# xiaopuren/KMC-with-a-diffusion-reaction-algorithm

Hardware: AMD Instinct MI355X
Metric: KMC particle-updates/sec (and steps/sec) at 1e6 particles, 1/2/4/8 MI355X (higher is better)
Workload: dtype f64

## Files before the change

kmc-with-a-diffusion-reaction-algorithm_amd/csrc/kmc_device.h:

```cpp
#pragma once
#include <hip/hip_runtime.h>
#include <stdint.h>

#include "kmc_math.h"
#include "kmc_philox.h"

namespace kmcd {

struct KParams {
  int NA, NB, N;
  int ncx, ncy;
  double gx0, gy0, cs;
  double box_x, box_y, box_z, pai;
  double ra, rb;
  double amp_a, amp_b, amp_cis, amp_bond;
  double rot_a, rot_b, rot_cis, rot_bond;
  double p_ass, p_mono, p_cis, p_diss, p_mdiss, p_cdiss;
  double bond_cut, cis_cut, thetapd_cut, thetaot_cut, cis_theta_cut;
  double T_aa, T_ab, T_bb, T_bond, T_cis;
  float ref_bb, ref_ab;
  int col_refine;
  float ref_rl;
  int rxn_refine;
  kmcr::Key key;
  int tcap;
  int tile;
  int dbg_stage;
  int tout_cap;
  int cx_serial;
  uint32_t cx_limit;
  int htag_max;
  int dbg_recs;
  int dbg_cand;
  int dd;
};

struct Ctl {
  uint32_t step;
  uint32_t obs_idx;
  uint32_t err;
  uint32_t err_step;
  uint32_t err_first;
  uint32_t n_overflow;
  uint32_t cx_cursor;
  uint32_t n_pend;
  uint32_t n_pqu, n_pqe;
  uint32_t n_cx;
  uint32_t n_heavy;
  uint32_t full_now;
  uint32_t n_dirty[2];
  uint32_t last[8];
  uint32_t n_rl;
  uint32_t n_cisc;
  uint32_t n_outl;
  uint32_t n_dense;
  int32_t off_bond, off_rl, off_cis, off_mono;
  int32_t maxc;
  uint32_t n_forced;
  uint32_t last_outl;
  uint32_t cand_kind[6];
  uint32_t rxn_kind[5];
  uint64_t vtag;
  uint64_t stamps[24];
  uint32_t dd_xcol, dd_xbond;
};

#define DD_JCAP 256
#define DD_XCAP 64
struct DDRep {
  int64_t xcol, xbond;
  int32_t bad, differed, links, n_jump, n_xb, reserved;
  int32_t jump_id[DD_JCAP];
  double jump_x[DD_JCAP];
  int32_t xb[DD_XCAP][2];
};

enum : uint32_t {
  ERR_EDGES = 1u,
  ERR_GEOMETRY = 2u,
  ERR_RESOLVE = 4u,
  ERR_ALIGN = 8u,
  ERR_MEMBERS = 16u,
  ERR_RECORDS = 32u,
};

enum : uint8_t { U_NONE = 0, U_FREE_A = 1, U_DIMER = 2, U_FREE_B = 3, U_COMPLEX = 4, U_DIMER_P = 5 };
enum : uint32_t { S_ACC = 1, S_PEND = 2, S_REJ = 3 };

#define ROWS_A 24
#define ROWS_B 12
#ifndef BEAD_BLOCK
#define BEAD_BLOCK 1
#endif
#ifndef BEAD_BS
#define BEAD_BS 64
#endif
#ifndef ROW_PERM
#define ROW_PERM 0
#endif
__host__ __device__ __forceinline__ int bead_row(int r, int rows) {
#if ROW_PERM
  constexpr unsigned char PA[24] = {0, 6, 7, 8, 1, 9, 10, 11, 2, 12, 13, 14, 3, 15, 16, 17, 4, 18, 19, 20, 5, 21, 22, 23};
  constexpr unsigned char PB[12] = {0, 6, 1, 7, 2, 8, 3, 9, 4, 10, 5, 11};
  return rows == 24 ? PA[r] : PB[r];
#else
  (void)rows;
  return r;
#endif
}
__host__ __device__ __forceinline__ size_t bead_elem(int i, int r, int n, int rows) {
#if BEAD_BLOCK
  (void)n;
  return ((size_t)(i / BEAD_BS) * rows + bead_row(r, rows)) * BEAD_BS + (i % BEAD_BS);
#else
  (void)rows;
  return (size_t)r * n + i;
#endif
}
__host__ __device__ __forceinline__ size_t bead_slots(int n) {
  return BEAD_BLOCK ? ((size_t)n + 63) / 64 * 64 : (size_t)n;
}
__host__ __device__ __forceinline__ size_t bead_off_a(int i, int j, int k, int c, int NA) {
  const int row = c < 2 ? (j - 1) * 4 + (k - 1) : 16 + ((j - 1) >> 1) * 4 + (k - 1);
  const int half = c < 2 ? c : ((j - 1) & 1);
  return bead_elem(i, row, NA, ROWS_A) * 2 + half;
}
__host__ __device__ __forceinline__ size_t bead_off_b(int i, int j, int k, int c, int NB) {
  const int row = c < 2 ? (j - 1) * 2 + (k - 1) : 8 + ((j - 1) >> 1) * 2 + (k - 1);
  const int half = c < 2 ? c : ((j - 1) & 1);
  return bead_elem(i, row, NB, ROWS_B) * 2 + half;
}
struct Beads {
  double* a;
  double* b;
  int NA, NB;
  __device__ __forceinline__ double& A(int i, int j, int k, int c) const { return a[bead_off_a(i, j, k, c, NA)]; }
  __device__ __forceinline__ double& B(int i, int j, int k, int c) const { return b[bead_off_b(i, j, k, c, NB)]; }
  __device__ __forceinline__ double2& A2(int i, int row) const {
    return reinterpret_cast<double2*>(a)[bead_elem(i, row, NA, ROWS_A)];
  }
  __device__ __forceinline__ double2& B2(int i, int row) const {
    return reinterpret_cast<double2*>(b)[bead_elem(i, row, NB, ROWS_B)];
  }
  __device__ __forceinline__ double2 Axy(int i, int j, int k) const { return A2(i, (j - 1) * 4 + (k - 1)); }
  __device__ __forceinline__ double2 Bxy(int i, int j, int k) const { return B2(i, (j - 1) * 2 + (k - 1)); }
  __device__ __forceinline__ double& P(int p, int j, int k, int c) const {
    return p < NA ? A(p, j, k, c) : B(p - NA, j, k, c);
  }
};

struct Rot {
  double t[3][3];
};
__device__ __forceinline__ Rot euler(double theta, double phi, double psai) {
  double cth = kmcm::cos(theta), sth = kmcm::sin(theta);
  double cph = kmcm::cos(phi), sph = kmcm::sin(phi);
  double cps = kmcm::cos(psai), sps = kmcm::sin(psai);
  Rot r;
  r.t[0][0] = cps * cph - cth * sph * sps;
  r.t[0][1] = -sps * cph - cth * sph * cps;
  r.t[0][2] = sth * sph;
  r.t[1][0] = cps * sph + cth * cph * sps;
  r.t[1][1] = -sps * sph + cth * cph * cps;
  r.t[1][2] = -sth * cph;
  r.t[2][0] = sps * sth;
  r.t[2][1] = cps * sth;
  r.t[2][2] = cth;
  return r;
}
__device__ __forceinline__ double rx(const Rot& r, double ox, double oy, double oz, double cx, double cy,
                                     double cz) {
  return r.t[0][0] * (ox - cx) + r.t[0][1] * (oy - cy) + r.t[0][2] * (oz - cz) + cx;
}
__device__ __forceinline__ double ry(const Rot& r, double ox, double oy, double oz, double cx, double cy,
                                     double cz) {
  return r.t[1][0] * (ox - cx) + r.t[1][1] * (oy - cy) + r.t[1][2] * (oz - cz) + cy;
}
__device__ __forceinline__ double rz(const Rot& r, double ox, double oy, double oz, double cx, double cy,
                                     double cz) {
  return r.t[2][0] * (ox - cx) + r.t[2][1] * (oy - cy) + r.t[2][2] * (oz - cz) + cz;
}

__device__ __forceinline__ double gettheta(double p0x, double p0y, double p0z, double p2x, double p2y,
                                           double p2z) {
  double lx0 = 0.0 - p0x, ly0 = 0.0 - p0y, lz0 = 0.0 - p0z;
  double lr0 = kmcm::sqrt_(lx0 * lx0 + ly0 * ly0 + lz0 * lz0);
  double lx1 = p2x - 0.0, ly1 = p2y - 0.0, lz1 = p2z - 0.0;
  double lr1 = kmcm::sqrt_(lx1 * lx1 + ly1 * ly1 + lz1 * lz1);
  double conv = 180 / 3.14159;
  double doth1 = -(lx1 * lx0 + ly0 * ly1 + lz0 * lz1);
  double doth2 = doth1 / (lr1 * lr0);
  if (doth2 > 1) doth2 = 1;
  if (doth2 < -1) doth2 = -1;
  return kmcm::acos(doth2) * conv;
}

__device__ __forceinline__ bool AreSame(double a, double b) { return kmcm::fabs_(a - b) < 1.0E-8; }

__device__ __forceinline__ double d2(double dx, double dy, double dz) { return dx * dx + dy * dy + dz * dz; }

__device__ __forceinline__ uint32_t ld_state(const uint32_t* p) {
  return __hip_atomic_load(p, __ATOMIC_RELAXED, __HIP_MEMORY_SCOPE_AGENT);
}
__device__ __forceinline__ void st_state(uint32_t* p, uint32_t v) {
  __hip_atomic_store(p, v, __ATOMIC_RELAXED, __HIP_MEMORY_SCOPE_AGENT);
}

}
```

kmc-with-a-diffusion-reaction-algorithm_amd/csrc/kmc_engine.hip:

```cpp
#include <hip/hip_runtime.h>

#include <algorithm>
#include <cmath>
#include <cstdio>
#include <cstdlib>
#include <cstring>
#include <string>
#include <vector>

#include "../../include/kmc.h"
#include "kmc_host.h"
#include "kmc_kernels.hip"
#include "kmc_analysis.hip"
#include "kmc_geometry.hip"
#include "kmc_structure.hip"
#include "kmc_dynamics.hip"

using namespace kmcd;

enum KId {
  KI_CLASSIFY, KI_BFS, KI_PROPOSE, KI_PROPOSE_FREE, KI_MOVE_MEMBERS, KI_CX_CHECK, KI_CX_HEAVY, KI_CX_KILL,
  KI_PAIR_SCAN, KI_COL_EXACT, KI_COL_ROUNDS, KI_COMMIT, KI_MATCH, KI_DISS_OBSERVE,
  KI_RESORT, KI_N
};
// ... 205 lines not shown
  rc |= dalloc(s, &d.dense, d.dense_cap);
  return rc;
}

double sqrt_threshold(double c) {
  double t = c * c;
  while (std::sqrt(t) >= c) t = std::nextafter(t, 0.0);
  while (std::sqrt(t) < c) t = std::nextafter(t, INFINITY);
  return t;
}


}

extern "C" {

const char* kmc_last_error(const kmc_sim* s) { return s ? s->err.c_str() : "null handle"; }

static int choose_tile(double rho) {
  int t = TILE_MAX;
  while (t > 4 && (t * t * rho > 205.0 || (t + 2) * (t + 2) * 2.0 * rho > 0.75 * TCAP)) --t;
  const char* te = getenv("KMC_TILE");
  if (te && *te) t = std::max(2, std::min(TILE_MAX, atoi(te)));
  return t;
}

int kmc_create(const kmc_params* p, int device, kmc_sim** out) {
  if (!p || !out) return KMC_ERR_ARG;
  *out = nullptr;
  if (p->n_a < 0 || p->n_b < 0 || p->n_a + p->n_b <= 0 || (int64_t)p->n_a + p->n_b > (1 << 24))
    return KMC_ERR_ARG;
  int ndev = 0;
  if (hipGetDeviceCount(&ndev) != hipSuccess || ndev == 0) return KMC_ERR_NODEVICE;
  kmc_sim* s = new kmc_sim();
  s->p = *p;
  if (device >= 0) {
    if (hipSetDevice(device) != hipSuccess) {
      delete s;
      return KMC_ERR_NODEVICE;
    }
    s->device = device;
  } else {
    (void)hipGetDevice(&s->device);
  }
  hipDeviceProp_t prop;
  if (hipGetDeviceProperties(&prop, s->device) != hipSuccess || std::strncmp(prop.gcnArchName, "gfx950", 6) != 0) {
    delete s;
    return KMC_ERR_NODEVICE;
  }
  if (hipStreamCreateWithFlags(&s->stream, hipStreamNonBlocking) != hipSuccess) {
    kmc_destroy(s);
    return KMC_ERR_HIP;
  }
  if (p->ra_radius > 20.0 || p->rb_radius > 30.0 || p->bond_dist_cutoff > 18.0 || p->cis_dist_cutoff > 15.0) {
    kmc_destroy(s);
    return KMC_ERR_ARG;
  }
  KParams& K = s->K;
  const int NA = p->n_a, NB = p->n_b, N = NA + NB;
  K.NA = NA;
  K.NB = NB;
  K.N = N;
  K.cs = 130.0;
  K.gx0 = -p->box_x / 2 - 1000.0;
  K.gy0 = -p->box_y / 2 - 1000.0;
  K.ncx = std::max(1, (int)((p->box_x + 2000.0) / K.cs) + 1);
  K.ncy = std::max(1, (int)((p->box_y + 2000.0) / K.cs) + 1);
  K.box_x = p->box_x;
  K.box_y = p->box_y;
  K.box_z = p->box_z;
  K.pai = p->pai;
  K.ra = p->ra_radius;
  K.rb = p->rb_radius;
  const double ts = p->time_step;
  K.amp_a = 2 * std::sqrt(p->ra_D * ts / 6);
  K.amp_b = 2 * std::sqrt(p->rb_D * ts / 6);
  K.amp_cis = 2 * std::sqrt(p->cis_D * ts / 6);
  K.amp_bond = 2 * std::sqrt(p->bond_D * ts / 6);
  K.rot_a = std::sqrt(p->ra_rot_D * ts);
  K.rot_b = std::sqrt(p->rb_rot_D * ts);
  K.rot_cis = std::sqrt(p->cis_rot_D * ts);
  K.rot_bond = std::sqrt(p->bond_rot_D * ts);
  K.p_ass = p->ass_rate * ts;
  K.p_mono = p->mono_cis_ass_rate * ts;
  K.p_cis = p->cis_ass_rate * ts;
  K.p_diss = p->diss_rate * ts;
  K.p_mdiss = p->mono_cis_diss_rate * ts;
  K.p_cdiss = p->cis_diss_rate * ts;
  K.bond_cut = p->bond_dist_cutoff;
  K.cis_cut = p->cis_dist_cutoff;
  K.thetapd_cut = p->bond_thetapd_cutoff;
  K.thetaot_cut = p->bond_thetaot_cutoff;
  K.cis_theta_cut = p->cis_thetaot_cutoff;
  K.T_aa = sqrt_threshold(p->ra_radius + p->ra_radius);
  K.T_ab = sqrt_threshold(p->ra_radius + p->rb_radius);
  K.T_bb = sqrt_threshold(p->rb_radius + p->rb_radius);
  K.T_bond = sqrt_threshold(p->bond_dist_cutoff);
  K.T_cis = sqrt_threshold(p->cis_dist_cutoff);
  K.ref_bb = (float)((2 * p->rb_radius + 2.5) * (2 * p->rb_radius + 2.5));
  K.ref_ab = (float)((p->ra_radius + p->rb_radius + 0.3 + 2.5) * (p->ra_radius + p->rb_radius + 0.3 + 2.5));
  K.ref_rl = (float)((p->bond_dist_cutoff + 3.0) * (p->bond_dist_cutoff + 3.0));
  {
    const char* cr = getenv("KMC_COL_REFINE");
    K.col_refine = !(cr && *cr == '0');
  }
  K.key = kmcr::make_key(p->seed, p->replica);

  s->ncell = 2 * K.ncx * K.ncy;
  Dev& d = s->d;
  d.cur.NA = d.nxt.NA = NA;
  d.cur.NB = d.nxt.NB = NB;
  d.nkeys = (uint32_t)N;
  int rc = KMC_OK;
  rc |= dalloc(s, &d.cur.a, 48 * bead_slots(NA));
  rc |= dalloc(s, &d.nxt.a, 48 * bead_slots(NA));
  rc |= dalloc(s, &d.cur.b, 24 * bead_slots(NB));
  rc |= dalloc(s, &d.nxt.b, 24 * bead_slots(NB));
  rc |= dalloc(s, &d.a_int, (size_t)5 * NA);
  rc |= dalloc(s, &d.b_int, (size_t)8 * NB);
  rc |= dalloc(s, &d.owner, N);
  rc |= dalloc(s, &d.id_of, N);
  rc |= dalloc(s, &d.slot_of, N);
  rc |= dalloc(s, &s->id_tmp, N);
  rc |= dalloc(s, &s->a_tmp, (size_t)5 * NA);
  rc |= dalloc(s, &s->b_tmp, (size_t)8 * NB);
  rc |= dalloc(s, &s->skeys, N);
  rc |= dalloc(s, &s->skeys2, N);
  rc |= dalloc(s, &s->svals, N);
  rc |= dalloc(s, &s->svals2, N);
  rc |= dalloc(s, &s->perm, N);
  rc |= dalloc(s, &s->newslot, N);
  rc |= dalloc(s, &d.ukind, N);
  rc |= dalloc(s, &d.ustate, N);
  rc |= dalloc(s, &d.moved, N);
  rc |= dalloc(s, &d.cx_off, NB);
  rc |= dalloc(s, &d.cx_size, NB);
  rc |= dalloc(s, &d.cx_nb, NB);
  rc |= dalloc(s, &d.cx_ext, NB);
  d.mcap = (uint32_t)(3 * (size_t)N);
  K.cx_limit = d.mcap / 2;
  {
    const char* cl = getenv("KMC_DEBUG_CX_LIMIT");
    if (cl && *cl) K.cx_limit = (uint32_t)std::max(0, std::min((int)K.cx_limit, atoi(cl)));
  }
  rc |= dalloc(s, &d.members, d.mcap);
  rc |= dalloc(s, &d.shuf, d.mcap);
  rc |= dalloc(s, &d.mrec, d.mcap);
  rc |= dalloc(s, &d.cxp, (size_t)NB * CXP);
  rc |= dalloc(s, &d.shuf_tag, NB);
  rc |= dalloc(s, &d.croot, N);
  rc |= dalloc(s, &d.cx_alive, NB);
  rc |= dalloc(s, &d.bfs_cand, NB);
  rc |= dalloc(s, &d.dlist, 2 * (size_t)N);
  rc |= dalloc(s, &d.pend, N);
  rc |= dalloc(s, &d.ccnt, N);
  rc |= dalloc(s, &d.overflow, NB);
  rc |= dalloc(s, &d.cx_list, (size_t)d.mcap / 2);
  rc |= dalloc(s, &d.cx_heavy, NB);
  rc |= dalloc(s, &s->hcnt, s->ncell + 1);
  {
    const size_t nblk = ((size_t)N + RS_TILE - 1) / RS_TILE;
    rc |= dalloc(s, &s->rs_cnt, 256 * nblk);
    rc |= dalloc(s, &s->rs_tot, 256);
    rc |= dalloc(s, &s->scan_part, ((size_t)s->ncell + 1 + SCAN_TILE - 1) / SCAN_TILE);
  }
  rc |= dalloc(s, &d.hstart, s->ncell + 1);
  rc |= dalloc(s, &d.home, N);
  rc |= dalloc(s, &d.rec, (size_t)2 * N);
  rc |= dalloc(s, &d.shard_cnt, (size_t)5 * NSHARD);
  {
    const char* cs = getenv("KMC_DEBUG_CAP_SHIFT");
    s->grow = cs && *cs ? -std::max(0, std::min(20, atoi(cs))) : 0;
  }
  rc |= alloc_lists(s);
  rc |= dalloc(s, &d.pq_units, N);
  rc |= dalloc(s, &d.obs_part, (size_t)8 * ((N + 255) / 256));
  rc |= dalloc(s, &d.bfs_queue, N);
  rc |= dalloc(s, &d.vtag, N);
  rc |= dalloc(s, &d.ctl, 1);
  if (rc != KMC_OK) {
    kmc_destroy(s);
    return KMC_ERR_HIP;
  }
  if (hipHostMalloc((void**)&s->ctl_host, sizeof(Ctl)) != hipSuccess) {
    kmc_destroy(s);
    return KMC_ERR_HIP;
  }
  const char* po = getenv("KMC_DEBUG_POISON");
  s->poison = po && *po == '1';
  const char* dc = getenv("KMC_DEBUG_COUNTS");
  s->debug_counts = dc && *dc == '1';
  const char* dsy = getenv("KMC_DEBUG_SYNC");
  s->debug_sync = dsy && *dsy == '1';
  const char* pc = getenv("KMC_DEBUG_PAIR_CHUNK");
  if (pc && *pc) s->an_chunk = std::max(1, std::min(AN_CHUNK, atoi(pc)));
  const char* tc = getenv("KMC_DEBUG_TCAP");
  K.tcap = TCAP;
  if (tc && *tc) K.tcap = std::max(0, std::min(TCAP, atoi(tc)));
  const char* oc = getenv("KMC_DEBUG_TOUT_CAP");
  K.tout_cap = TOUT_CAP;
  if (oc && *oc) K.tout_cap = std::max(0, std::min(TOUT_CAP, atoi(oc)));
  {
    K.tile = choose_tile((double)N * K.cs * K.cs / std::max(1.0, p->box_x * p->box_y));
    const char* fb = getenv("KMC_FULL_BFS");
    s->always_full = fb && *fb == '1';
    const char* ds = getenv("KMC_DEBUG_SCAN_STAGE");
    K.dbg_stage = ds && *ds ? atoi(ds) : 0;
    const char* cxs = getenv("KMC_CX_SERIAL");
    K.cx_serial = cxs && *cxs == '1';
    const char* gr = getenv("KMC_GRAPH");
    s->use_graphs = gr && *gr == '1';
    const char* cs = getenv("KMC_CX_STREAM");
    s->cx_stream = (cs && *cs) ? std::max(0, std::min(3, atoi(cs))) : ((int64_t)N >= CX_STREAM_N ? 3 : 0);
    const char* cpw = getenv("KMC_CX_PARAMS_WG");
    s->cx_params_wg = cpw && *cpw ? std::max(0, atoi(cpw)) : 0;
    const char* ht = getenv("KMC_DEBUG_HTAG");
    K.htag_max = HTAG_MAX;
    if (ht && *ht) K.htag_max = std::max(0, std::min(HTAG_MAX, atoi(ht)));
    const char* dca = getenv("KMC_DEBUG_CAND");
    K.dbg_cand = dca && *dca == '1';
    const char* dr = getenv("KMC_DEBUG_RECS");
    K.dbg_recs = dr && *dr == '1';
    if (K.dbg_recs && dalloc(s, &d.rec_step, 2 * (size_t)N) != KMC_OK) {
      kmc_destroy(s);
      return KMC_ERR_HIP;
    }
    const char* sp = getenv("KMC_SNAP_SPAN");
    if (sp && *sp) s->snap_span = std::max<int64_t>(0, atoll(sp));
  }
  {
    const uint64_t kmax = (uint64_t)K.ncx * K.ncy;
    s->key_bits = 1;
    while ((1ull << s->key_bits) < kmax) ++s->key_bits;
    if (s->key_bits + 33 > 64) {
      kmc_destroy(s);
      return KMC_ERR_ARG;
    }
    const char* re = getenv("KMC_RESORT");
    if (re && *re) s->resort_every = atoll(re);
    const char* gs = getenv("KMC_GROUP_SORT");
    if (gs && *gs) s->group_sort = std::max(0, std::min(2, atoi(gs)));
    s->ntiles = ((K.ncx + K.tile - 1) / K.tile) * ((K.ncy + K.tile - 1) / K.tile);
    if (dalloc(s, &s->d.tout, (size_t)s->ntiles * TOUT_CAP) != KMC_OK ||
        dalloc(s, &s->d.tout_n, (size_t)s->ntiles) != KMC_OK) {
      kmc_destroy(s);
      return KMC_ERR_HIP;
    }
  }
  *out = s;
  return KMC_OK;
}

int kmc_destroy(kmc_sim* s) {
  if (!s) return KMC_OK;
  if (s->stream) (void)hipStreamSynchronize(s->stream);
  for (void* v : s->allocs) (void)hipFree(v);
  if (s->obs_buf) (void)hipFree(s->obs_buf);
  if (s->ctl_host) (void)hipHostFree(s->ctl_host);
  for (auto& e : s->tev)
    if (e) (void)hipEventDestroy(e);
  for (auto& g : s->graphs)
    if (g.exec) (void)hipGraphExecDestroy(g.exec);
  if (s->side) (void)hipStreamSynchronize(s->side);
  for (auto& e : s->an_ev)
    if (e) (void)hipEventDestroy(e);
  if (s->ev_fork) (void)hipEventDestroy(s->ev_fork);
  if (s->ev_join) (void)hipEventDestroy(s->ev_join);
  if (s->side) (void)hipStreamDestroy(s->side);
  if (s->stream) (void)hipStreamDestroy(s->stream);
  delete s;
  return KMC_OK;
}

int64_t kmc_current_step(const kmc_sim* s) { return s ? s->step_done : -1; }

static void reorder(kmc_sim* s, const int32_t* perm, const int32_t* map, bool swap_in) {
  const KParams& K = s->K;
  Dev& d = s->d;
  hipStream_t st = s->stream;
  const int NA = K.NA, NB = K.NB, T = 256, mode = swap_in ? 0 : 1;
  auto g = [&](size_t n) { return (unsigned)((n + T - 1) / T); };
  if (NA > 0) {
    k_gather_beads<<<g((size_t)(swap_in ? ROWS_A : 48) * NA), T, 0, st>>>(d.cur.a, d.nxt.a, perm, 0, NA, 0, mode);
    k_gather_i32<<<g((size_t)5 * NA), T, 0, st>>>(d.a_int, s->a_tmp, perm, 0, NA, 5, (1u << 2) | (1u << 4), map);
  }
  if (NB > 0) {
    k_gather_beads<<<g((size_t)(swap_in ? ROWS_B : 24) * NB), T, 0, st>>>(d.cur.b, d.nxt.b, perm, NA, NB, 1, mode);
    k_gather_i32<<<g((size_t)8 * NB), T, 0, st>>>(d.b_int, s->b_tmp, perm, NA, NB, 8, 0xf0u, map);
  }
  if (!swap_in) return;
  std::swap(d.cur.a, d.nxt.a);
  std::swap(d.cur.b, d.nxt.b);
  std::swap(d.a_int, s->a_tmp);
  std::swap(d.b_int, s->b_tmp);
}

__global__ void k_iota(int32_t* a, int32_t* b, int n) {
  int i = blockIdx.x * blockDim.x + threadIdx.x;
  if (i < n) a[i] = b[i] = i;
}

static void dev_scan(kmc_sim* s, const int32_t* in, int32_t* out, int n, hipStream_t st) {
  const int nb = (n + SCAN_TILE - 1) / SCAN_TILE;
  k_scan_part<<<nb, 256, 0, st>>>(in, n, s->scan_part);
  k_scan_top<<<1, 256, 0, st>>>(s->scan_part, nb);
  k_scan_down<<<nb, 256, 0, st>>>(in, out, n, s->scan_part);
}

static int32_t* radix_sort(kmc_sim* s, int nbits, hipStream_t st, uint64_t** keys_out) {
  const int N = s->K.N, nblk = (N + RS_TILE - 1) / RS_TILE;
  uint64_t *ka = s->skeys, *kb = s->skeys2;
  int32_t *va = s->svals, *vb = s->svals2;
  if (nblk == 0) nbits = 0;
  for (int shift = 0; shift < nbits; shift += 8) {
    k_rs_hist<<<nblk, 256, 0, st>>>(ka, N, shift, s->rs_cnt, nblk);
    k_rs_rows<<<256, 256, 0, st>>>(s->rs_cnt, nblk, s->rs_tot);
    k_rs_scatter<<<nblk, 256, 0, st>>>(ka, va, kb, vb, N, shift, s->rs_cnt, s->rs_tot, nblk);
    std::swap(ka, kb);
    std::swap(va, vb);
  }
  *keys_out = ka;
  return va;
}

static int check_sort(kmc_sim* s, const uint64_t* dk, const int32_t* dv) {
  const int N = s->K.N, NA = s->K.NA;
  std::vector<uint64_t> k((size_t)N);
  std::vector<int32_t> v((size_t)N);
  HIPCHK(s, hipStreamSynchronize(s->stream));
  HIPCHK(s, hipMemcpy(k.data(), dk, sizeof(uint64_t) * N, hipMemcpyDeviceToHost));
  HIPCHK(s, hipMemcpy(v.data(), dv, sizeof(int32_t) * N, hipMemcpyDeviceToHost));
  std::vector<uint8_t> seen((size_t)N, 0);
  for (int i = 0; i < N; ++i) {
    const int kind = i >= NA, base = kind ? NA : 0, nk = kind ? N - NA : NA;
    if (v[i] < 0 || v[i] >= nk || seen[(size_t)base + v[i]]++)
      return fail(s, KMC_ERR_HIP, "KMC_DEBUG_SYNC: re-sort values not a permutation at " + std::to_string(i));
    if (i > 0 && (k[i] < k[i - 1] || (k[i] == k[i - 1] && v[i] <= v[i - 1])))
      return fail(s, KMC_ERR_HIP, "KMC_DEBUG_SYNC: re-sort keys out of order at " + std::to_string(i));
  }
  return KMC_OK;
}

static int home_build(kmc_sim* s) {
  const KParams& K = s->K;
  Dev& d = s->d;
  hipStream_t st = s->stream;
  const int N = K.N, T = 256;
  HIPCHK(s, hipMemsetAsync(s->hcnt, 0, sizeof(int32_t) * (size_t)(s->ncell + 1), st));
  k_home_count<<<(N + T - 1) / T, T, 0, st>>>(K, d, s->hcnt);
  dev_scan(s, s->hcnt, d.hstart, s->ncell + 1, st);
  if (s->debug_sync) {
    const size_t n = (size_t)s->ncell + 1;
    std::vector<int32_t> c(n), h(n);
    HIPCHK(s, hipStreamSynchronize(st));
    HIPCHK(s, hipMemcpy(c.data(), s->hcnt, sizeof(int32_t) * n, hipMemcpyDeviceToHost));
    HIPCHK(s, hipMemcpy(h.data(), d.hstart, sizeof(int32_t) * n, hipMemcpyDeviceToHost));
    int64_t run = 0;
    for (size_t i = 0; i < n; ++i) {
      if (h[i] != run) return fail(s, KMC_ERR_HIP, "KMC_DEBUG_SYNC: home scan wrong at " + std::to_string(i));
      run += c[i];
    }
  }
  k_home_place<<<(N + T - 1) / T, T, 0, st>>>(K, d);
  return hipGetLastError() == hipSuccess ? KMC_OK : fail(s, KMC_ERR_HIP, "home_build launch");
}

// ... 188 lines not shown

int kmc_load_cpt(kmc_sim* s, const char* path) {
  if (!s || !path) return KMC_ERR_ARG;
  const int NA = s->p.n_a, NB = s->p.n_b;
  std::vector<double> ra((size_t)48 * NA + 1), rb((size_t)24 * NB + 1);
  std::vector<int32_t> ai((size_t)5 * NA + 1), bi((size_t)8 * NB + 1);
  kmc_state_view v{ra.data(), rb.data(), ai.data(), bi.data(), {0, 0, 0, 0, 0}, 0, 0};
  int rc = kmch_host::load_cpt(&s->p, path, &v, &s->err);
  if (rc != KMC_OK) return rc;
  return kmc_set_state(s, &v);
}

int kmc_write_cpt(kmc_sim* s, const char* path) {
  if (!s || !path) return KMC_ERR_ARG;
  const int NA = s->p.n_a, NB = s->p.n_b;
  std::vector<double> ra((size_t)48 * NA + 1), rb((size_t)24 * NB + 1);
  std::vector<int32_t> ai((size_t)5 * NA + 1), bi((size_t)8 * NB + 1);
  kmc_state_view v{ra.data(), rb.data(), ai.data(), bi.data(), {0, 0, 0, 0, 0}, 0, 0};
  int rc = kmc_get_state(s, &v);
  if (rc != KMC_OK) return rc;
  return kmch_host::write_cpt(&s->p, &v, path, &s->err);
}

int kmc_save_state(kmc_sim* s, const char* path) {
  if (!s || !path) return KMC_ERR_ARG;
  const int NA = s->p.n_a, NB = s->p.n_b;
  std::vector<double> ra((size_t)48 * NA + 1), rb((size_t)24 * NB + 1);
  std::vector<int32_t> ai((size_t)5 * NA + 1), bi((size_t)8 * NB + 1);
  kmc_state_view v{ra.data(), rb.data(), ai.data(), bi.data(), {0, 0, 0, 0, 0}, 0, 0};
  int rc = kmc_get_state(s, &v);
  if (rc != KMC_OK) return rc;
  return kmch_host::save_state(&s->p, &v, path, &s->err);
}

int kmc_load_state(kmc_sim* s, const char* path) {
  if (!s || !path) return KMC_ERR_ARG;
  const int NA = s->p.n_a, NB = s->p.n_b;
  std::vector<double> ra((size_t)48 * NA + 1), rb((size_t)24 * NB + 1);
  std::vector<int32_t> ai((size_t)5 * NA + 1), bi((size_t)8 * NB + 1);
  kmc_state_view v{ra.data(), rb.data(), ai.data(), bi.data(), {0, 0, 0, 0, 0}, 0, 0};
  int rc = kmch_host::load_state(&s->p, path, &v, &s->err);
  if (rc != KMC_OK) return rc;
  return kmc_set_state(s, &v);
}

static void harvest(kmc_sim* s, int slot) {
  for (int k = 0; k < KI_N; ++k) {
    size_t i = (size_t)slot * KI_N + k;
    if (!s->tused[i]) continue;
    float ms = 0;
    (void)hipEventSynchronize(s->tev[2 * i + 1]);
    if (hipEventElapsedTime(&ms, s->tev[2 * i], s->tev[2 * i + 1]) == hipSuccess) {
      s->kms[k] += ms;
      s->kcount[k] += 1;
    }
    s->tused[i] = 0;
  }
}

struct Bracket {
  kmc_sim* s;
  int k;
  hipStream_t st;
  Bracket(kmc_sim* s_, int k_, hipStream_t st_) : s(s_), k(k_), st(st_) {
    if (s->tnow && (s->tmask >> k & 1)) (void)hipEventRecord(s->tev[2 * ((size_t)s->tslot * KI_N + k)], st);
  }
  ~Bracket() {
    if (s->tnow && (s->tmask >> k & 1)) {
      size_t i = (size_t)s->tslot * KI_N + k;
      (void)hipEventRecord(s->tev[2 * i + 1], st);
      s->tused[i] = 1;
    }
  }
};
#define TIMED(k, ...) TIMED_ON(k, s->stream, __VA_ARGS__)
#define TIMED_ON(k, STREAM, ...)                                                                        \
  do {                                                                                                  \
    {                                                                                                   \
      Bracket b_(s, k, STREAM);                                                                         \
      __VA_ARGS__;                                                                                      \
    }                                                                                                   \
    if (s->debug_sync) {                                                                                \
      const hipError_t e_ = hipStreamSynchronize(STREAM);                                               \
      if (e_ != hipSuccess)                                                                             \
        return fail(s, KMC_ERR_HIP, std::string("KMC_DEBUG_SYNC: ") + KNAMES[k] + " failed in step " +     \
                                        std::to_string(s->launch_base) + ": " + hipGetErrorString(e_)); \
    }                                                                                                   \
  } while (0)

static int debug_check_lists(kmc_sim* s) {
  Dev& d = s->d;
  const int N = s->K.N;
  HIPCHK(s, hipStreamSynchronize(s->stream));
  std::vector<uint32_t> cnt(5 * NSHARD);
  HIPCHK(s, hipMemcpy(cnt.data(), d.shard_cnt, sizeof(uint32_t) * cnt.size(), hipMemcpyDeviceToHost));
  const SList* L[5] = {&d.cand, &d.conf, &d.plist, &d.rej, &d.pairs};
  const char* names[5] = {"cand", "conf", "plist", "rej", "pairs"};
  char m[300];
  for (int l = 0; l < 5; ++l) {
    std::vector<int2> v((size_t)L[l]->cap * NSHARD);
    HIPCHK(s, hipMemcpy(v.data(), L[l]->data, sizeof(int2) * v.size(), hipMemcpyDeviceToHost));
    for (int k = 0; k < NSHARD; ++k) {
      const uint32_t c = std::min(cnt[l * NSHARD + k], L[l]->cap);
      for (uint32_t t = 0; t < c; ++t) {
        const int2 e = v[(size_t)k * L[l]->cap + t];
        const int x = e.x, y = l == 1 ? (e.y & 0x7fffffff) : e.y;
        bool ok = true;
        if (l == 0 || l == 4) ok = x >= 0 && x < 2 * N && y >= 0 && y < 2 * N;
        if (l == 1) ok = x >= 0 && x < N && y >= 0 && y < N;
        if (l == 2 || l == 3) ok = x >= 0 && x < N;
        if (!ok) {
          snprintf(m, sizeof m, "KMC_DEBUG_SYNC: list %s shard %d entry %u = (%d, %d) out of range (N %d) in step %lld",
                   names[l], k, t, e.x, e.y, N, (long long)s->launch_base);
          return fail(s, KMC_ERR_HIP, m);
        }
      }
    }
  }
  return KMC_OK;
}

#ifndef COARSE_N
#define COARSE_N (4 << 20)
#endif
static int side_stream(kmc_sim* s) {
  if (s->side) return KMC_OK;
  int lo = 0, hi = 0;
  const char* pr = getenv("KMC_CX_STREAM_PRIO");
  const bool prio = !(pr && *pr == '0') && hipDeviceGetStreamPriorityRange(&lo, &hi) == hipSuccess;
  if ((prio ? hipStreamCreateWithPriority(&s->side, hipStreamNonBlocking, hi)
            : hipStreamCreateWithFlags(&s->side, hipStreamNonBlocking)) != hipSuccess ||
      hipEventCreateWithFlags(&s->ev_fork, hipEventDisableTiming) != hipSuccess ||
      hipEventCreateWithFlags(&s->ev_join, hipEventDisableTiming) != hipSuccess)
    return fail(s, KMC_ERR_HIP, "the complexes' stream");
  return KMC_OK;
}

static int launch_step(kmc_sim* s, bool re_sort) {
  const KParams& K = s->K;
  Dev& d = s->d;
  hipStream_t st = s->stream;
  const int T = 256;
  const int gN = (K.N + T - 1) / T, gB = (K.NB + T - 1) / T;
  if (s->tnow) harvest(s, s->tslot);
  if (re_sort) {
    int rc;
    TIMED(KI_RESORT, rc = resort(s));
    if (rc != KMC_OK) return rc;
  }
  if (s->poison) {
    (void)hipMemsetAsync(d.nxt.a, 0xff, sizeof(double) * 48 * bead_slots(K.NA), st);
    (void)hipMemsetAsync(d.nxt.b, 0xff, sizeof(double) * 24 * bead_slots(K.NB), st);
  }
  if (K.NB > 0 && (s->need_full || re_sort || s->always_full))
    TIMED(KI_CX_KILL, (k_cx_kill<<<std::min(gN, 1024), T, 0, st>>>(K, d)));
  s->need_full = false;
  const int per = K.N >= COARSE_N ? 4 : 1, gP = (K.N + T * per - 1) / (T * per);
  if (per == 4) TIMED(KI_CLASSIFY, (k_classify<4><<<gP, T, 0, st>>>(K, d)));
  else TIMED(KI_CLASSIFY, (k_classify<1><<<gP, T, 0, st>>>(K, d)));
  {
    Bracket b_(s, KI_PROPOSE, st);
    const int gL = std::min(2048, (K.NB + T - 1) / T);
    const bool side = s->cx_stream != 0 && K.NB > 0 && !s->use_graphs;
    if (K.NB > 0 && (!side || s->cx_stream == 3)) {
      TIMED(KI_BFS, (k_bfs<<<gB, T, 0, st>>>(K, d)));
    }
    const int gC = K.NB > 0 ? std::min(gL, 512) : 0;
    const int gP3 = s->cx_params_wg > 0 ? std::min(s->cx_params_wg, 1 << 16) : gL;
    if (side && s->cx_stream == 3) {
      const int rc = side_stream(s);
      if (rc != KMC_OK) return rc;
      hipStream_t sd = s->side;
      k_propose_free<<<gP3, T, 0, st>>>(K, d, gP3);
      TIMED(KI_MOVE_MEMBERS, (k_move_members<<<gN, T, 0, st>>>(K, d)));
      HIPCHK(s, hipEventRecord(s->ev_fork, st));
      HIPCHK(s, hipStreamWaitEvent(sd, s->ev_fork, 0));
      TIMED_ON(KI_CX_CHECK, sd, (k_cx_check<<<gL, T, 0, sd>>>(K, d)));
      TIMED_ON(KI_CX_HEAVY, sd, (k_complex_heavy<<<1024, T, 0, sd>>>(K, d)));
      HIPCHK(s, hipEventRecord(s->ev_join, sd));
      TIMED(KI_PROPOSE_FREE, (k_propose_free<<<gN, T, 0, st>>>(K, d, 0)));
      HIPCHK(s, hipStreamWaitEvent(st, s->ev_join, 0));
    } else if (side) {
      const int rc = side_stream(s);
      if (rc != KMC_OK) return rc;
      hipStream_t sd = s->side;
      HIPCHK(s, hipEventRecord(s->ev_fork, st));
      HIPCHK(s, hipStreamWaitEvent(sd, s->ev_fork, 0));
      TIMED_ON(KI_BFS, sd, (k_bfs<<<gB, T, 0, sd>>>(K, d)));
      k_propose_free<<<gC, T, 0, sd>>>(K, d, gC);
      if (s->cx_stream == 1) {
        TIMED_ON(KI_MOVE_MEMBERS, sd, (k_move_members<<<gN, T, 0, sd>>>(K, d)));
        TIMED_ON(KI_CX_CHECK, sd, (k_cx_check<<<gL, T, 0, sd>>>(K, d)));
        TIMED_ON(KI_CX_HEAVY, sd, (k_complex_heavy<<<1024, T, 0, sd>>>(K, d)));
      }
      HIPCHK(s, hipEventRecord(s->ev_join, sd));
      TIMED(KI_PROPOSE_FREE, (k_propose_free<<<gN, T, 0, st>>>(K, d, 0)));
      HIPCHK(s, hipStreamWaitEvent(st, s->ev_join, 0));
      if (s->cx_stream == 2) {
        TIMED(KI_MOVE_MEMBERS, (k_move_members<<<gN, T, 0, st>>>(K, d)));
        TIMED(KI_CX_CHECK, (k_cx_check<<<gL, T, 0, st>>>(K, d)));
        TIMED(KI_CX_HEAVY, (k_complex_heavy<<<1024, T, 0, st>>>(K, d)));
      }
    } else {
      TIMED(KI_PROPOSE_FREE, (k_propose_free<<<gC + gN, T, 0, st>>>(K, d, gC)));
      if (K.NB > 0) {
        TIMED(KI_MOVE_MEMBERS, (k_move_members<<<gN, T, 0, st>>>(K, d)));
        TIMED(KI_CX_CHECK, (k_cx_check<<<gL, T, 0, st>>>(K, d)));
        TIMED(KI_CX_HEAVY, (k_complex_heavy<<<1024, T, 0, st>>>(K, d)));
      }
    }
  }
  if (K.dbg_recs) k_rec_check<<<std::min(2048, (2 * K.N + T - 1) / T), T, 0, st>>>(K, d);
  const int gX = std::min(2048, (K.N + T - 1) / T);
  const int ntiles = s->ntiles;
  TIMED(KI_PAIR_SCAN, (k_pair_scan<<<ntiles, PAIR_THREADS, 0, st>>>(K, d)));
  TIMED(KI_COL_EXACT, {
#if DENSE_KERNEL
    k_col_dense<<<64, T, 0, st>>>(K, d);
    if (s->debug_sync && hipStreamSynchronize(st) != hipSuccess)
      return fail(s, KMC_ERR_HIP, "KMC_DEBUG_SYNC: k_col_dense failed in step " + std::to_string(s->launch_base));
#endif
    k_col_exact<<<std::max(gX, 64), T, 0, st>>>(K, d);
  });
  if (s->debug_sync) {
    const int rc = debug_check_lists(s);
    if (rc != KMC_OK) return rc;
  }
  TIMED(KI_COL_ROUNDS, {
    k_col_resolve<<<gX, T, 0, st>>>(K, d);
    if (s->debug_sync && hipStreamSynchronize(st) != hipSuccess)
      return fail(s, KMC_ERR_HIP, "KMC_DEBUG_SYNC: k_col_resolve failed in step " + std::to_string(s->launch_base));
    k_col_tail<<<1, 1024, 0, st>>>(K, d, 1);
  });
#ifndef COMMIT_RXN
#define COMMIT_RXN 1
#endif
#if COMMIT_RXN
  TIMED(KI_COMMIT, (k_commit_rxn<<<gX + (K.NA > 0 ? 1024 : 0), T, 0, st>>>(K, d, gX)));
#else
  TIMED(KI_COMMIT, {
    k_commit_rxn<<<gX, T, 0, st>>>(K, d, gX);
    if (K.NA > 0) k_commit_rxn<<<1024, T, 0, st>>>(K, d, 0);
  });
#endif
  if (K.NA > 0) TIMED(KI_MATCH, (k_match<<<1, 1024, 0, st>>>(K, d)));
  TIMED(KI_DISS_OBSERVE, {
    if (per == 4) k_diss_observe<4><<<gP, T, 0, st>>>(K, d);
    else k_diss_observe<1><<<gP, T, 0, st>>>(K, d);
    k_finalize<<<1, 1024, 0, st>>>(K, d, s->p.time_step, gP);
  });
  if (s->tnow) s->tslot = (s->tslot + 1) % TRING;
  std::swap(d.cur, d.nxt);
  return KMC_OK;
}

static int launch_step_graph(kmc_sim* s) {
  unsigned char key[sizeof(KParams) + sizeof(Dev)];
  std::memcpy(key, &s->K, sizeof(KParams));
  std::memcpy(key + sizeof(KParams), &s->d, sizeof(Dev));
  for (auto& g : s->graphs)
    if (g.valid && std::memcmp(g.key, key, sizeof key) == 0) {
      HIPCHK(s, hipGraphLaunch(g.exec, s->stream));
      std::swap(s->d.cur, s->d.nxt);
      ++s->graph_launches;
      return KMC_OK;
    }
  auto& g = s->graphs[s->graph_next];
  s->graph_next = (s->graph_next + 1) % kmc_sim::NGRAPH;
  if (g.exec) (void)hipGraphExecDestroy(g.exec);
  g.exec = nullptr;
  g.valid = false;
  HIPCHK(s, hipStreamBeginCapture(s->stream, hipStreamCaptureModeThreadLocal));
  const int rc = launch_step(s, false);
  hipGraph_t graph = nullptr;
  const hipError_t ec = hipStreamEndCapture(s->stream, &graph);
  if (rc != KMC_OK) {
    if (graph) (void)hipGraphDestroy(graph);
    return rc;
  }
  HIPCHK(s, ec);
  const hipError_t ei = hipGraphInstantiate(&g.exec, graph, nullptr, nullptr, 0);
  (void)hipGraphDestroy(graph);
  HIPCHK(s, ei);
  std::memcpy(g.key, key, sizeof key);
  g.valid = true;
  ++s->graph_captures;
  HIPCHK(s, hipGraphLaunch(g.exec, s->stream));
  ++s->graph_launches;
  return KMC_OK;
}

static int dd_after_step(kmc_sim* s);

static int run_chunk(kmc_sim* s, int64_t n, int64_t base, kmc_obs* out = nullptr) {
  HIPCHK(s, hipMemsetAsync(&s->d.ctl->obs_idx, 0, sizeof(uint32_t), s->stream));
  for (int64_t k = 0; k < n; ++k) {
    const bool rs = s->resort_every > 0 && ++s->since_resort >= s->resort_every;
    if (rs) s->since_resort = 0;
    if (((base + k + 1) & 0x3fffffff) == 0)
      HIPCHK(s, hipMemsetAsync(s->d.ustate, 0, sizeof(uint32_t) * (size_t)s->K.N, s->stream));
    s->tnow = s->tmask && (s->tcount++ % s->tperiod) == 0;
    const bool plain = !rs && !s->tnow && !s->poison && !s->need_full && !s->always_full &&
                       s->K.dbg_stage == 0 && !s->debug_sync;
    s->launch_base = base + k + 1;
    int rc = (s->use_graphs && plain) ? launch_step_graph(s) : launch_step(s, rs);
    if (rc != KMC_OK) return rc;
  }
  HIPCHK(s, hipGetLastError());
  if (s->dd_step_pending) {
    const int rc = dd_after_step(s);
    if (rc != KMC_OK) return rc;
  }
  HIPCHK(s, hipMemcpyAsync(s->ctl_host, s->d.ctl, sizeof(Ctl), hipMemcpyDeviceToHost, s->stream));
  if (out) HIPCHK(s, hipMemcpyAsync(out, s->obs_buf, sizeof(kmc_obs_dev) * n, hipMemcpyDeviceToHost, s->stream));
  HIPCHK(s, hipStreamSynchronize(s->stream));
  if (s->tmask)
    for (int slot = 0; slot < TRING; ++slot) harvest(s, slot);
  return KMC_OK;
}

int kmc_step(kmc_sim* s, int64_t nsteps, kmc_obs* out) {
  if (!s) return KMC_ERR_ARG;
  if (!s->have_state) return fail(s, KMC_ERR_ARG, "no state: call kmc_init_random / kmc_load_cpt / kmc_set_state");
  if (nsteps <= 0) return KMC_OK;
  static_assert(sizeof(kmc_obs_dev) == sizeof(kmc_obs), "obs layout");
  const int64_t chunk = 4096;
  if (!s->obs_buf) {
    HIPCHK(s, hipMalloc((void**)&s->obs_buf, sizeof(kmc_obs_dev) * chunk));
    s->obs_cap = chunk;
    s->d.obs = s->obs_buf;
  }
  int64_t done = 0;
  while (done < nsteps) {
    const int64_t n = std::min(chunk, nsteps - done);
    int rc = KMC_OK;
    if (!s->K.dd && (!s->snap_valid || s->step_done + n - s->snap_step > s->snap_span)) {
      rc = snapshot(s, false);
      if (rc != KMC_OK) return rc;
      s->snap_valid = true;
      s->snap_step = s->step_done;
      s->snap_since = s->since_resort;
      ++s->n_snapshots;
    }
    bool copied = false;
    for (;;) {
      rc = run_chunk(s, n, s->step_done, out ? out + done : nullptr);
      if (rc != KMC_OK) return rc;
      const uint32_t err = s->ctl_host->err;
      if (!err) {
        copied = out != nullptr;
        break;
      }
      const uint32_t cause = s->ctl_host->err_first;
      const int64_t bad = (int64_t)s->ctl_host->err_step;
      if (s->K.dd) {
        const bool grow = (cause & ~ERR_EDGES) == 0;
        if (grow && s->grow < 6) {
          s->grow += 1;
          if (alloc_lists(s) != KMC_OK) return fail(s, KMC_ERR_HIP, "growing the output lists failed");
        }
        s->have_state = false;
        s->clusters_valid = false;
        char m[200];
        snprintf(m, sizeof m, "dd: device error bits 0x%x at step %lld; the window's state is lost (list growth 2^%d)",
                 err, (long long)bad, s->grow);
        return fail(s, grow ? KMC_ERR_CAPACITY : (cause & ERR_GEOMETRY) ? KMC_ERR_GEOMETRY : KMC_ERR_CAPACITY, m);
      }
      rc = snapshot(s, true);
      if (rc != KMC_OK) return rc;
      s->since_resort = s->snap_since;
      s->need_full = true;
      ++s->n_replays;
      const bool grow = (cause & ~ERR_EDGES) == 0 && s->grow < 6;
      if (grow) {
        s->grow += 1;
        if (alloc_lists(s) != KMC_OK) return fail(s, KMC_ERR_HIP, "growing the output lists failed");
      }
      for (int64_t at = s->snap_step; at < s->step_done;) {
        const int64_t m = std::min(chunk, s->step_done - at);
        rc = run_chunk(s, m, at);
        if (rc != KMC_OK) return rc;
        if (s->ctl_host->err) {
          rc = snapshot(s, true);
          if (rc != KMC_OK) {
            s->have_state = false;
            return rc;
          }
          const int64_t at_fail = at;
          s->step_done = s->snap_step;
          s->since_resort = s->snap_since;
          s->need_full = true;
          s->clusters_valid = false;
          char m2[200];
          snprintf(m2, sizeof m2,
                   "replay from the snapshot raised an error the original steps did not (in steps %lld..%lld); "
                   "state restored to step %lld",
                   (long long)at_fail + 1, (long long)(at_fail + m), (long long)s->step_done);
          return fail(s, KMC_ERR_HIP, m2);
        }
        at += m;
      }
      if (grow) continue;
      const int64_t good = std::max<int64_t>(0, std::min<int64_t>(n, bad - (s->step_done + 1)));
      if (good > 0) {
        rc = run_chunk(s, good, s->step_done);
        if (rc != KMC_OK) return rc;
        if (out)
          HIPCHK(s, hipMemcpy(out + done, s->obs_buf, sizeof(kmc_obs_dev) * good, hipMemcpyDeviceToHost));
        s->step_done += good;
      }
      s->clusters_valid = good > 0;
      char m[200];
      snprintf(m, sizeof m, "device error bits 0x%x at step %lld; state kept at step %lld", err, (long long)bad,
               (long long)s->step_done);
      const int code = (cause & ERR_GEOMETRY) ? KMC_ERR_GEOMETRY : KMC_ERR_CAPACITY;
      return fail(s, code, m);
    }
    if (out && !copied)
      HIPCHK(s, hipMemcpy(out + done, s->obs_buf, sizeof(kmc_obs_dev) * n, hipMemcpyDeviceToHost));
    s->step_done += n;
    s->clusters_valid = true;
    if (s->debug_counts) {
      const uint32_t* l = s->ctl_host->last;
      fprintf(stderr, "kmc step %lld: candidates %u conflicts %u pending-units %u rejected %u rxn-pairs %u rl-edges %u cis-edges %u bfs-overflow %u outliers %u (list growth 2^%d, replays %lld, snapshots %lld, forced rebuilds %u)\n",
              (long long)s->step_done, l[0], l[1], l[2], l[3], l[4], l[5], l[6], l[7], s->ctl_host->last_outl, s->grow,
              (long long)s->n_replays, (long long)s->n_snapshots, s->ctl_host->n_forced);
      if (s->K.dbg_cand) {
        const uint32_t* c = s->ctl_host->cand_kind;
        const uint32_t* r = s->ctl_host->rxn_kind;
        fprintf(stderr, "kmc cand AA %u/%u AB %u/%u BB %u/%u (tested/colliding) rxn %u final %u gate %u accept %u "
                "refined-out %u\n",
                c[0], c[1], c[2], c[3], c[4], c[5], r[0], r[1], r[2], r[3], r[4]);
      }
#if WALK_STATS
      {
        unsigned long long w = 0, wo = 0;
        if (hipMemcpyFromSymbol(&w, HIP_SYMBOL(kmc_walk_pairs), sizeof w) == hipSuccess &&
            hipMemcpyFromSymbol(&wo, HIP_SYMBOL(kmc_walk_pairs_old), sizeof wo) == hipSuccess)
          fprintf(stderr, "kmc walk pairs %llu old-position items %llu (summed since the library loaded)\n", w, wo);
      }
#endif
      const uint64_t* t = s->ctl_host->stamps;
      if (t[16])
        fprintf(stderr, "kmc stamps heavy stage %llu align %llu writeback %llu records %llu (cycles summed over "
                "waves) complexes %llu max-cycles %llu members %llu\n",
                (unsigned long long)t[16], (unsigned long long)t[17], (unsigned long long)t[18],
                (unsigned long long)t[19], (unsigned long long)t[20], (unsigned long long)t[21],
                (unsigned long long)t[22]);
      if (t[0] | t[8])
        fprintf(stderr, "kmc stamps col %llu %llu %llu %llu %llu %llu %llu %llu rxn %llu %llu %llu %llu %llu %llu %llu %llu\n",
                (unsigned long long)t[0], (unsigned long long)t[1], (unsigned long long)t[2], (unsigned long long)t[3],
                (unsigned long long)t[4], (unsigned long long)t[5], (unsigned long long)t[6], (unsigned long long)t[7],
                (unsigned long long)t[8], (unsigned long long)t[9], (unsigned long long)t[10], (unsigned long long)t[11],
                (unsigned long long)t[12], (unsigned long long)t[13], (unsigned long long)t[14], (unsigned long long)t[15]);
    }
    done += n;
  }
  return KMC_OK;
}

__global__ void k_math(int op, const double* x, const double* y, double* out, int n) {
  int i = blockIdx.x * blockDim.x + threadIdx.x;
  if (i >= n) return;
  double a = x[i], b = y[i], r = 0;
  switch (op) {
    case 0: r = kmcm::sin(a); break;
    case 1: r = kmcm::cos(a); break;
    case 2: r = kmcm::atan2(a, b); break;
    case 3: r = kmcm::acos(a); break;
    case 4: r = kmcm::sqrt_(a); break;
    case 5: r = a / b; break;
    default: r = kmcm::round_(a); break;
  }
  out[i] = r;
}

int kmc_device_math(int op, const double* x, const double* y, double* out, int64_t n) {
  if (n <= 0) return KMC_OK;
  double *dx = nullptr, *dy = nullptr, *dout = nullptr;
  size_t b = sizeof(double) * (size_t)n;
  if (hipMalloc(&dx, b) != hipSuccess || hipMalloc(&dy, b) != hipSuccess || hipMalloc(&dout, b) != hipSuccess)
    return KMC_ERR_HIP;
  int rc = KMC_OK;
  if (hipMemcpy(dx, x, b, hipMemcpyHostToDevice) != hipSuccess || hipMemcpy(dy, y, b, hipMemcpyHostToDevice) != hipSuccess)
    rc = KMC_ERR_HIP;
  if (rc == KMC_OK) {
    k_math<<<(int)((n + 255) / 256), 256>>>(op, dx, dy, dout, (int)n);
    if (hipDeviceSynchronize() != hipSuccess || hipMemcpy(out, dout, b, hipMemcpyDeviceToHost) != hipSuccess)
      rc = KMC_ERR_HIP;
  }
  (void)hipFree(dx);
  (void)hipFree(dy);
  (void)hipFree(dout);
  return rc;
}

int kmc_get_clusters(kmc_sim* s, int32_t* row_len, int32_t* members) {
  if (!s || !row_len || !members) return KMC_ERR_ARG;
  if (!s->have_state || !s->clusters_valid)
    return fail(s, KMC_ERR_ARG, "no step simulated since the state was set (or the last chunk was undone)");
  const int NA = s->p.n_a, NB = s->p.n_b, N = NA + NB;
  std::vector<uint8_t> kind(N);
  std::vector<int32_t> off(NB), size(NB), mem(N), id_of(N), slot_of(N);
  HIPCHK(s, hipStreamSynchronize(s->stream));
  HIPCHK(s, hipMemcpy(kind.data(), s->d.ukind, N, hipMemcpyDeviceToHost));
  HIPCHK(s, hipMemcpy(off.data(), s->d.cx_off, sizeof(int32_t) * NB, hipMemcpyDeviceToHost));
  HIPCHK(s, hipMemcpy(size.data(), s->d.cx_size, sizeof(int32_t) * NB, hipMemcpyDeviceToHost));
  std::vector<int32_t> shuf(s->d.mcap);
  std::vector<uint32_t> stag(NB);
  mem.resize(s->d.mcap);
  HIPCHK(s, hipMemcpy(mem.data(), s->d.members, sizeof(int32_t) * s->d.mcap, hipMemcpyDeviceToHost));
  HIPCHK(s, hipMemcpy(shuf.data(), s->d.shuf, sizeof(int32_t) * s->d.mcap, hipMemcpyDeviceToHost));
  HIPCHK(s, hipMemcpy(stag.data(), s->d.shuf_tag, sizeof(uint32_t) * NB, hipMemcpyDeviceToHost));
  HIPCHK(s, hipMemcpy(id_of.data(), s->d.id_of, sizeof(int32_t) * N, hipMemcpyDeviceToHost));
  HIPCHK(s, hipMemcpy(slot_of.data(), s->d.slot_of, sizeof(int32_t) * N, hipMemcpyDeviceToHost));
  int64_t o = 0;
  for (int b = 0; b < NB; ++b) {
    int p = slot_of[NA + b];
    if (kind[p] == U_FREE_B) {
      row_len[b] = 1;
      members[o++] = NA + b + 1;
    } else if (kind[p] == U_COMPLEX) {
      int lb = p - NA;
      row_len[b] = size[lb];
      const int32_t* row = (stag[lb] == (uint32_t)s->step_done ? shuf.data() : mem.data()) + off[lb];
      for (int t = 0; t < size[lb]; ++t) members[o++] = id_of[row[t]] + 1;
    } else {
      row_len[b] = 0;
    }
  }
  return KMC_OK;
}

int kmc_set_timing(kmc_sim* s, uint64_t kernel_mask) {
  if (!s) return KMC_ERR_ARG;
  if (kernel_mask && s->tev.empty()) {
    s->tev.assign((size_t)TRING * KI_N * 2, nullptr);
    s->tused.assign((size_t)TRING * KI_N, 0);
    for (auto& e : s->tev) HIPCHK(s, hipEventCreate(&e));
  }
  s->tmask = kernel_mask;
  s->tcount = 0;
  for (int k = 0; k < KI_N; ++k) {
    s->kms[k] = 0;
    s->kcount[k] = 0;
  }
  return KMC_OK;
}

int kmc_set_timing_period(kmc_sim* s, int32_t every) {
  if (!s || every < 1) return KMC_ERR_ARG;
  s->tperiod = every;
  return KMC_OK;
}

int kmc_kernel_times(const kmc_sim* s, double* total_ms, int64_t* launches, int32_t n) {
  if (!s) return KMC_ERR_ARG;
  for (int k = 0; k < n && k < KI_N; ++k) {
    if (total_ms) total_ms[k] = s->kms[k];
    if (launches) launches[k] = s->kcount[k];
  }
  return KI_N;
}

const char* kmc_kernel_name(int32_t id) { return id >= 0 && id < KI_N ? KNAMES[id] : ""; }

}

__global__ void k_dd_export(KParams P, Dev d, int n, const int32_t* ids, double* beads, int32_t* ints) {
  const int NA = P.NA, NB = P.NB;
  const size_t t = (size_t)blockIdx.x * blockDim.x + threadIdx.x;
  if (t < (size_t)n * 48) {
    const int i = (int)(t / 48), e = (int)(t % 48), slot = d.slot_of[ids[i]], bead = e / 3, c = e % 3;
    double v = 0.0;
    if (slot < NA) v = d.cur.A(slot, bead / 4 + 1, bead % 4 + 1, c);
    else if (e < 24) v = d.cur.B(slot - NA, bead / 2 + 1, bead % 2 + 1, c);
    beads[t] = v;
  }
  if (t < (size_t)n * 8) {
    const int i = (int)(t / 8), f = (int)(t % 8), slot = d.slot_of[ids[i]];
    int v = 0;
    bool link = false;
    if (slot < NA) {
      if (f < 5) v = d.a_int[(size_t)f * NA + slot];
      link = f == 2 || f == 4;
    } else {
      v = d.b_int[(size_t)f * NB + (slot - NA)];
      link = f >= 4;
    }
    if (link && v > 0) v = d.id_of[v - 1] + 1;
    ints[t] = v;
  }
}

__global__ void k_dd_import(KParams P, Dev d, int n, const int32_t* ids, const double* beads, const int32_t* ints,
                            uint8_t* flags) {
  const int NA = P.NA, NB = P.NB;
  const size_t t = (size_t)blockIdx.x * blockDim.x + threadIdx.x;
  if (t < (size_t)n * 48) {
    const int i = (int)(t / 48), e = (int)(t % 48), slot = d.slot_of[ids[i]], bead = e / 3, c = e % 3;
    double* dst = nullptr;
    if (slot < NA) dst = &d.cur.A(slot, bead / 4 + 1, bead % 4 + 1, c);
    else if (e < 24) dst = &d.cur.B(slot - NA, bead / 2 + 1, bead % 2 + 1, c);
    if (dst) {
      const double v = beads[t];
      if (__double_as_longlong(*dst) != __double_as_longlong(v)) {
        atomicOr((uint32_t*)&flags[i & ~3], 1u << (8 * (i & 3)));
        *dst = v;
      }
    }
  }
  if (t < (size_t)n * 8) {
    const int i = (int)(t / 8), f = (int)(t % 8), slot = d.slot_of[ids[i]];
    int32_t* dst = nullptr;
    bool link = false;
    if (slot < NA) {
      if (f < 5) dst = &d.a_int[(size_t)f * NA + slot];
      link = f == 2 || f == 4;
    } else {
      dst = &d.b_int[(size_t)f * NB + (slot - NA)];
      link = f >= 4;
    }
    if (dst) {
      int v = ints[t];
      if (link && v > 0) v = d.slot_of[v - 1] + 1;
      if (*dst != v) {
        atomicOr((uint32_t*)&flags[i & ~3], 2u << (8 * (i & 3)));
        *dst = v;
      }
    }
  }
}

__global__ void k_dd_drift(KParams P, Dev d, uint32_t* out) {
  const int p = blockIdx.x * blockDim.x + threadIdx.x;
  float m = 0.0f;
  if (p < P.N) {
    const int r = d.id_of[p];
    if (d.dd_own[r]) {
      double dx = d.cur.P(p, 1, 1, 0) - d.dd_x0[r];
      dx = dx - P.box_x * kmcm::round_(dx / P.box_x);
      m = (float)kmcm::fabs_(dx);
    }
  }
  for (int o = 32; o > 0; o >>= 1) m = fmaxf(m, __shfl_down(m, o, 64));
  if (__lane_id() == 0) atomicMax(out, __float_as_uint(m));
}

__global__ void k_dd_jumpers(KParams P, Dev d, double S, int cap, int32_t* ids, double* xs, uint32_t* cnt) {
  const int p = blockIdx.x * blockDim.x + threadIdx.x;
  if (p >= P.N) return;
  const int r = d.id_of[p];
  if (!d.dd_own[r]) return;
  const double x = d.cur.P(p, 1, 1, 0);
  double dx = x - d.dd_x0[r];
  dx = dx - P.box_x * kmcm::round_(dx / P.box_x);
  if (!(kmcm::fabs_(dx) > S)) return;
  const uint32_t k = atomicAdd(cnt, 1u);
// ... 989 lines not shown
```

kmc-with-a-diffusion-reaction-algorithm_amd/csrc/kmc_kernels.hip:

```cpp
#include "kmc_device.h"

namespace kmcd {

#ifndef NSHARD
#define NSHARD 64
#endif
struct SList {
  int2* data;
  uint32_t* cnt;
  uint32_t cap;
};

struct Dev {
  Beads cur, nxt;
  int32_t* a_int;
  int32_t* b_int;
  int32_t* owner;
  int32_t* id_of;
  int32_t* slot_of;
  uint8_t* ukind;
  uint32_t* ustate;
  uint32_t* moved;
  int32_t* cx_off;
  int32_t* cx_size;
  int32_t* cx_nb;
  uint32_t* cx_ext;
  int32_t* members;
  int32_t* shuf;
  int4* mrec;
  double* cxp;
  uint32_t* shuf_tag;
  uint32_t mcap;
  int32_t* croot;
  uint32_t* cx_alive;
  uint32_t* bfs_cand;
  int32_t* dlist;
  uint32_t* pend;
  unsigned long long* ccnt;
  int32_t* overflow;
  int4* cx_list;
  int4* cx_heavy;
  uint2* home;
  int32_t* hstart;
  struct Rec* rec;
  int4* outl;
  uint32_t outl_cap;
  int2* tout;
  uint32_t* tout_n;
  uint32_t* rec_step;
  int4* dense;
  uint32_t dense_cap;
  SList cand;
  SList conf;
  SList plist;
  SList rej;
  SList pairs;
  int32_t* pq_units;
  int2* pq_ent;
  uint32_t* shard_cnt;
  int32_t* obs_part;
  uint64_t* rl_keys;
  uint64_t* cis_keys;
  uint64_t* ent;
  int32_t* gi32;
  uint32_t cap_edges;
  int32_t* bfs_queue;
  uint32_t* vtag;
  Ctl* ctl;
  struct kmc_obs_dev* obs;
  const int32_t* gid;
  const uint8_t* dd_own;
  const double* dd_x0;
  DDRep* dd_rep;
  uint32_t nkeys;
};

struct alignas(16) Rec {
  float4 pos;
  int2 id;
  float2 site;
};
#define RID_PID 0x00ffffff
#define RID_LIG (1 << 24)
#define RID_CODE_SHIFT 25
#define RID_OUT 15
#define RID_ST3 (1 << 29)
#define RID_ST2 (1 << 30)
__device__ __forceinline__ int rec_code(int2 id) { return (id.x >> RID_CODE_SHIFT) & 15; }

struct kmc_obs_dev {
  int64_t step;
  double t;
  int32_t rl, mono, cis, bond;
  double cluster_size;
  int32_t maxc, tot_prot, tot_clu, reserved;
};

#define A_ST2(d, i) (d).a_int[0 * (size_t)NA + (i)]
#define A_ST3(d, i) (d).a_int[1 * (size_t)NA + (i)]
#define A_NEI2(d, i) (d).a_int[2 * (size_t)NA + (i)]
#define A_NEI4(d, i) (d).a_int[3 * (size_t)NA + (i)]
#define A_NEI3(d, i) (d).a_int[4 * (size_t)NA + (i)]
#define B_ST(d, b, j) (d).b_int[(size_t)((j)-1) * NB + (b)]
#define B_NEI(d, b, j) (d).b_int[(size_t)(4 + (j)-1) * NB + (b)]

__device__ __forceinline__ bool bad_key(const Dev& d, int key) {
  if ((uint32_t)key < d.nkeys) return false;
  atomicOr(&d.ctl->err, ERR_RESOLVE);
  return true;
}
__device__ __forceinline__ uint32_t state_of(const Dev& d, int key, uint32_t step) {
  if (bad_key(d, key)) return S_REJ;
  uint32_t v = ld_state(&d.ustate[key]);
  return (v >> 2) == (step & 0x3fffffffu) ? (v & 3u) : S_ACC;
}
__device__ __forceinline__ void set_state(const Dev& d, int key, uint32_t step, uint32_t s) {
  if (bad_key(d, key)) return;
  st_state(&d.ustate[key], ((step & 0x3fffffffu) << 2) | s);
}

__device__ __forceinline__ uint32_t rkey(const KParams& P, const Dev& d, int r) {
  return P.dd ? (uint32_t)d.gid[r] : (uint32_t)r;
}
__device__ __forceinline__ bool dd_owned(const KParams& P, const Dev& d, int r) { return !P.dd || d.dd_own[r]; }
__device__ __forceinline__ void dd_xbond(const Dev& d, int a, int b) {
  if (d.dd_own[a] == d.dd_own[b]) return;
  atomicAdd(&d.ctl->dd_xbond, 1u);
  const uint32_t k = atomicAdd((uint32_t*)&d.dd_rep->n_xb, 1u);
  if (k < DD_XCAP) {
    d.dd_rep->xb[k][0] = a;
    d.dd_rep->xb[k][1] = b;
  }
}

__device__ __forceinline__ int cell_x(const KParams& P, double x) {
  int c = (int)__builtin_floor((x - P.gx0) / P.cs);
  return c < 0 ? 0 : (c >= P.ncx ? P.ncx - 1 : c);
}
__device__ __forceinline__ int cell_y(const KParams& P, double y) {
  int c = (int)__builtin_floor((y - P.gy0) / P.cs);
  return c < 0 ? 0 : (c >= P.ncy ? P.ncy - 1 : c);
}

#define CROOT_BIG (1 << 30)
#define CXL 16

__device__ __forceinline__ uint32_t wave_slot(uint32_t* ctr) {
  const uint64_t mask = __ballot(1);
  const int lane = __lane_id();
  const int leader = __ffsll((unsigned long long)mask) - 1;
  const uint32_t rank = __popcll(mask & ((1ull << lane) - 1ull));
  uint32_t base = 0;
  if (lane == leader) base = atomicAdd(ctr, (uint32_t)__popcll(mask));
  base = __shfl(base, leader, 64);
  return base + rank;
}

__device__ __forceinline__ uint32_t wave_alloc(uint32_t* ctr, uint32_t qn) {
  const uint64_t mask = __ballot(1);
  const int lane = __lane_id(), leader = __ffsll((unsigned long long)mask) - 1;
  uint32_t pre = 0, tot = 0;
  for (uint64_t m = mask; m; m &= m - 1) {
    const int l = __ffsll((unsigned long long)m) - 1;
    const uint32_t v = (uint32_t)__shfl((int)qn, l, 64);
    pre += l < lane ? v : 0u;
    tot += v;
  }
  uint32_t base = 0;
  if (lane == leader) base = atomicAdd(ctr, tot);
  return (uint32_t)__shfl((int)base, leader, 64) + pre;
}

template <int CLASSIFY_PER>
__global__ void k_classify(KParams P, Dev d) {
  const int NA = P.NA, NB = P.NB;
  const int p0 = blockIdx.x * blockDim.x * CLASSIFY_PER + threadIdx.x;
  int n2[CLASSIFY_PER], n3[CLASSIFY_PER], s2[CLASSIFY_PER], r[CLASSIFY_PER];
#pragma unroll
  for (int k = 0; k < CLASSIFY_PER; ++k) {
    const int p = p0 + k * (int)blockDim.x;
    n2[k] = n3[k] = s2[k] = 0;
    r[k] = -1;
    if (p >= P.N) continue;
    if (p < NA) {
      n2[k] = A_NEI2(d, p);
      n3[k] = A_NEI3(d, p);
      s2[k] = A_ST2(d, p) | A_ST3(d, p);
    } else {
      const int b = p - NA;
      n2[k] = B_NEI(d, b, 2);
      n3[k] = B_NEI(d, b, 3);
      s2[k] = B_NEI(d, b, 4);
    }
    r[k] = d.croot[p];
    if (r[k] >= 0) r[k] &= ~CROOT_BIG;
  }
#pragma unroll
  for (int k = 0; k < CLASSIFY_PER; ++k) {
    const int p = p0 + k * (int)blockDim.x;
    if (p >= P.N) continue;
    uint8_t kind = U_NONE;
    int own = -1;
    if (p < NA) {
      const int i = p;
      if (s2[k] == 0) {
        kind = U_FREE_A;
        own = p;
      } else if (n2[k] == 0 && n3[k] != 0 && A_NEI3(d, n3[k] - 1) == i + 1 && A_NEI2(d, n3[k] - 1) == 0) {
        int q = n3[k] - 1;
        const bool lead = d.id_of[i] < d.id_of[q];
        own = lead ? i : q;
        kind = lead ? U_DIMER : U_DIMER_P;
      }
    } else if (n2[k] == 0 && n3[k] == 0 && s2[k] == 0) {
      kind = U_FREE_B;
      own = p;
    }
    if (r[k] >= 0) {
      own = r[k];
      if (r[k] == p) kind = U_COMPLEX;
    }
    d.ukind[p] = kind;
    d.owner[p] = own < 0 ? -1 : d.id_of[own];
  }
}

__device__ __forceinline__ void cx_reset_all(const KParams& P, const Dev& d, uint32_t tid, uint32_t nt) {
  for (uint32_t p = tid; p < (uint32_t)P.N; p += nt) d.croot[p] = -1;
  for (uint32_t b = tid; b < (uint32_t)P.NB; b += nt) d.cx_alive[b] = 0;
  if (tid == 0) {
    d.ctl->cx_cursor = 0;
    d.ctl->n_cx = 0;
    d.ctl->full_now = 1;
  }
}
__global__ void k_cx_kill(KParams P, Dev d) {
  cx_reset_all(P, d, blockIdx.x * blockDim.x + threadIdx.x, gridDim.x * blockDim.x);
}
__device__ __forceinline__ void cx_dissolve_dirty(const KParams& P, const Dev& d, uint32_t step) {
  const int NA = P.NA;
  const uint32_t li = step & 1, n = min(d.ctl->n_dirty[li], (uint32_t)P.N), next = step + 1;
  for (uint32_t t = threadIdx.x; t < n; t += blockDim.x) {
    const int p = d.dlist[(size_t)li * P.N + t];
    if (p >= NA) d.bfs_cand[p - NA] = next;
    const int r = d.croot[p] & ~CROOT_BIG;
    if (r < 0 || atomicExch(&d.cx_alive[r - NA], 0u) != 1u) continue;
    const int b = r - NA, off = d.cx_off[b], sz = d.cx_size[b];
    for (int i = 0; i < sz; ++i) {
      const int m = d.members[off + i];
      d.croot[m] = -1;
      if (m >= NA) d.bfs_cand[m - NA] = next;
    }
  }
}

__device__ __forceinline__ void mark_bond_change(const KParams& P, const Dev& d, int p, uint32_t step) {
  if (P.NB == 0) return;
  const uint32_t li = step & 1;
  const uint32_t t = atomicAdd(&d.ctl->n_dirty[li], 1u);
  if (t < (uint32_t)P.N) d.dlist[(size_t)li * P.N + t] = p;
}

#define BFS_QCAP 32
#ifndef BFS_BATCH
#define BFS_BATCH 4
#endif

__device__ __forceinline__ void nbrs3(const KParams& P, const Dev& d, int x, int* y) {
  const int NA = P.NA, NB = P.NB;
  if (x < NA) {
    const int a = A_NEI2(d, x), b = A_NEI3(d, x);
    y[0] = a > 0 ? a - 1 : (b > 0 ? b - 1 : -1);
    y[1] = a > 0 && b > 0 ? b - 1 : -1;
    y[2] = -1;
  } else {
    const int lb = x - NA;
    const int v2 = B_NEI(d, lb, 2), v3 = B_NEI(d, lb, 3), v4 = B_NEI(d, lb, 4);
    y[0] = v2 > 0 ? v2 - 1 : -1;
    y[1] = v3 > 0 ? v3 - 1 : -1;
    y[2] = v4 > 0 ? v4 - 1 : -1;
  }
}

#define CXD_MOVED (1 << 30)
#define CXD_LB 0x3fffffff

template <int STRIDE = 1>
__device__ __forceinline__ void register_complex(const KParams& P, const Dev& d, int p, const int* q, int qn) {
  const int NA = P.NA, NB = P.NB;
  uint32_t off = wave_alloc(&d.ctl->cx_cursor, (uint32_t)qn);
  if (off + qn > d.mcap) {
    atomicOr(&d.ctl->err, ERR_MEMBERS);
    qn = 0;
    off = 0;
  }
  int nb = 0;
  const int rootid = d.id_of[p];
#pragma unroll 4
  for (int t = 0; t < qn; ++t) {
    int m = q[t * STRIDE];
    d.members[off + t] = m;
    d.owner[m] = rootid;
    d.croot[m] = p | (qn > CXL ? CROOT_BIG : 0);
    nb += m >= NA;
  }
  d.cx_alive[p - NA] = 1;
  if (qn <= CXL) {
    auto enc = [&](int v) -> int {
      if (v <= 0) return 0;
      for (int t = 0; t < qn; ++t)
        if (q[t * STRIDE] == v - 1) return (v - 1 < NA ? t : NA + t) + 1;
      atomicOr(&d.ctl->err, ERR_RESOLVE);
      return 0;
    };
    for (int t0 = 0; t0 < qn; t0 += 4) {
      int4 r[4];
#pragma unroll
      for (int i = 0; i < 4; ++i) {
        const int t = t0 + i, m = t < qn ? q[t * STRIDE] : p;
        r[i].x = m;
        if (m < NA) {
          r[i].y = A_NEI2(d, m);
          r[i].z = A_NEI3(d, m);
          r[i].w = A_NEI4(d, m);
        } else {
          r[i].y = B_NEI(d, m - NA, 2);
          r[i].z = B_NEI(d, m - NA, 3);
          r[i].w = B_NEI(d, m - NA, 4);
        }
      }
#pragma unroll
      for (int i = 0; i < 4; ++i) {
        if (t0 + i >= qn) break;
        r[i].y = enc(r[i].y);
        r[i].z = enc(r[i].z);
        if (r[i].x >= NA) r[i].w = enc(r[i].w);
        d.mrec[off + t0 + i] = r[i];
      }
    }
  }
  int b = p - NA;
  d.cx_off[b] = (int)off;
  d.cx_size[b] = qn;
  d.cx_nb[b] = nb;
  d.ukind[p] = U_COMPLEX;
  const int4 desc = make_int4(b, (int)off, qn | nb << 16, rootid);
  const uint32_t slot = wave_slot(&d.ctl->n_cx);
  if (slot < d.mcap / 2) d.cx_list[slot] = desc;
  else atomicOr(&d.ctl->err, ERR_MEMBERS);
}

__global__ void __launch_bounds__(256) k_bfs(KParams P, Dev d) {
  __shared__ int qs[BFS_QCAP * 256];
  const int NA = P.NA, NB = P.NB;
  int b = blockIdx.x * blockDim.x + threadIdx.x;
  if (b >= NB) return;
  if (!d.ctl->full_now && d.bfs_cand[b] != d.ctl->step) return;
  if (B_NEI(d, b, 2) == 0 && B_NEI(d, b, 3) == 0 && B_NEI(d, b, 4) == 0) return;
  int* q = qs + threadIdx.x;
  int p = NA + b;
  const int pid = d.id_of[p];
  auto lower = [&](int qn) {
    bool lw = false;
    for (int t0 = 1; t0 < qn; t0 += 8) {
      int id[8];
#pragma unroll
      for (int i = 0; i < 8; ++i) {
        const int t = t0 + i, v = t < qn ? q[t * 256] : 0;
        id[i] = v >= NA ? d.id_of[v] : pid;
      }
#pragma unroll
      for (int i = 0; i < 8; ++i) lw |= id[i] < pid;
    }
    return lw;
  };
  int qn = 1, head = 0;
  q[0] = p;
  uint64_t bloom = 1ull << (((uint32_t)p * 0x9E3779B1u) >> 26);
  while (head < qn) {
    const int nb = min(BFS_BATCH, qn - head);
    int y[BFS_BATCH][3];
#pragma unroll
    for (int i = 0; i < BFS_BATCH; ++i)
      if (i < nb) nbrs3(P, d, q[(head + i) * 256], y[i]);
#pragma unroll
    for (int i = 0; i < BFS_BATCH; ++i) {
      if (i >= nb) break;
#pragma unroll
      for (int e = 0; e < 3; ++e) {
        int v = y[i][e];
        if (v < 0) continue;
        const uint64_t bit = 1ull << (((uint32_t)v * 0x9E3779B1u) >> 26);
        if (bloom & bit) {
          bool seen = false;
          for (int t = 0; t < qn; ++t) seen |= q[t * 256] == v;
          if (seen) continue;
        }
        bloom |= bit;
        if (qn == BFS_QCAP) {
          if (lower(qn) || (v >= NA && d.id_of[v] < pid)) return;
          uint32_t s = atomicAdd(&d.ctl->n_overflow, 1u);
          d.overflow[s] = b;
          return;
        }
        q[(qn++) * 256] = v;
      }
    }
    head += nb;
  }
  if (lower(qn)) return;
  register_complex<256>(P, d, p, q, qn);
}

__device__ __forceinline__ int bfs_overflow_one(const KParams& P, const Dev& d, uint32_t o) {
  const int NA = P.NA;
  int p = NA + d.overflow[o];
  const int pid = d.id_of[p];
  uint32_t tag = (uint32_t)(++d.ctl->vtag);
  int* q = d.bfs_queue;
  int qn = 0, head = 0;
  q[qn++] = p;
  d.vtag[p] = tag;
  while (head < qn) {
    int x = q[head++];
    int y[3];
    nbrs3(P, d, x, y);
#pragma unroll
    for (int e = 0; e < 3; ++e) {
      int v = y[e];
      if (v < 0) continue;
      if (v >= NA && d.id_of[v] < pid) return -1;
      if (d.vtag[v] == tag) continue;
      d.vtag[v] = tag;
      q[qn++] = v;
    }
  }
  register_complex(P, d, p, q, qn);
  return p - NA;
}

typedef double kmc_dbl2v __attribute__((ext_vector_type(2)));
__device__ __forceinline__ double2 ld_r(const double2& r) {
  const kmc_dbl2v v = __builtin_nontemporal_load(reinterpret_cast<const kmc_dbl2v*>(&r));
  return make_double2(v.x, v.y);
}
__device__ __forceinline__ void st_n(double2& r, double2 v) {
  kmc_dbl2v w;
  w.x = v.x;
  w.y = v.y;
  __builtin_nontemporal_store(w, reinterpret_cast<kmc_dbl2v*>(&r));
}

__device__ __forceinline__ void ref_point(const Dev& d, const Beads& B, int p, int NA, double& x, double& y,
                                          double& zlo, double& zhi) {
  if (p < NA) {
    const double2 xy = B.Axy(p, 1, 1), z12 = B.A2(p, 16), z34 = B.A2(p, 20);
    x = xy.x;
    y = xy.y;
    double z1 = z12.x, z2 = z12.y, z3 = z34.x, z4 = z34.y;
    zlo = fmin(fmin(z1, z2), fmin(z3, z4));
    zhi = fmax(fmax(z1, z2), fmax(z3, z4));
  } else {
    const double2 xy = B.Bxy(p - NA, 1, 1);
    x = xy.x;
    y = xy.y;
    zlo = B.B(p - NA, 1, 1, 2);
    zhi = zlo;
  }
}

__device__ __forceinline__ bool extent_ok(const Beads& B, int p, int NA) {
  if (p < NA) {
    double x0 = B.A(p, 1, 1, 0), y0 = B.A(p, 1, 1, 1);
    for (int j = 2; j <= 4; ++j) {
      double dx = B.A(p, j, 1, 0) - x0, dy = B.A(p, j, 1, 1) - y0;
      if (!(dx * dx + dy * dy <= 0.09)) return false;
    }
    return true;
  }
  int b = p - NA;
  double x0 = B.B(b, 1, 1, 0), y0 = B.B(b, 1, 1, 1);
  for (int j = 2; j <= 4; ++j) {
    double dx = B.B(b, j, 1, 0) - x0, dy = B.B(b, j, 1, 1) - y0;
    if (!(dx * dx + dy * dy <= 35.0 * 35.0)) return false;
  }
  return true;
}

__device__ __forceinline__ int cell_index(const KParams& P, int cx, int cy, int kind) {
  return (cy * 2 + kind) * P.ncx + cx;
}

#ifndef TOUT_CAP
#define TOUT_CAP 64
#endif
__device__ __forceinline__ void tile_bucket_push(const KParams& P, const Dev& d, int ri, int cx, int cy) {
  const int t = P.tile, ntx = (P.ncx + t - 1) / t;
  const int tx = cx / t, ty = cy / t, rx = cx - tx * t, ry = cy - ty * t;
  const int x0 = tx - (rx == 0 && tx > 0 ? 1 : 0), x1 = tx + (rx == t - 1 && (tx + 1) * t < P.ncx ? 1 : 0);
  const int y0 = ty - (ry == 0 && ty > 0 ? 1 : 0), y1 = ty + (ry == t - 1 && (ty + 1) * t < P.ncy ? 1 : 0);
  for (int y = y0; y <= y1; ++y)
    for (int x = x0; x <= x1; ++x) {
      const int b = y * ntx + x;
      const uint32_t o = atomicAdd(&d.tout_n[b], 1u);
      if (o < (uint32_t)P.tout_cap) d.tout[(size_t)b * TOUT_CAP + o] = make_int2(ri, cx | cy << 16);
    }
}

__device__ __forceinline__ void put_rec_raw(const KParams& P, const Dev& d, uint2 h, int p, int w, int st, int own,
                                            double x, double y, float4 pos, float2 site) {
  const int cx = cell_x(P, x), cy = cell_y(P, y);
  const int dx = cx - (int)(h.y & 0xffffu), dy = cy - (int)(h.y >> 16);
  const int ri = 2 * (int)h.x + w;
  int code = RID_OUT;
  if (dx >= -1 && dx <= 1 && dy >= -1 && dy <= 1) {
    code = (dy + 1) * 3 + (dx + 1);
  } else {
    const uint32_t o = atomicAdd(&d.ctl->n_outl, 1u);
    if (o < d.outl_cap) d.outl[o] = make_int4(ri, cx, cy, 0);
    else atomicOr(&d.ctl->err, ERR_EDGES);
    tile_bucket_push(P, d, ri, cx, cy);
  }
  Rec r;
  r.pos = pos;
  r.id = make_int2(p | (p >= P.NA ? RID_LIG : 0) | code << RID_CODE_SHIFT | st | (w << 31), own);
  r.site = site;
  d.rec[ri] = r;
  if (P.dbg_recs) d.rec_step[ri] = d.ctl->step;
}
__device__ __forceinline__ void put_rec(const KParams& P, const Dev& d, uint2 h, int p, int w, int st, int own,
                                        double x, double y, double zlo, double zhi, double sx, double sy) {
  put_rec_raw(P, d, h, p, w, st, own, x, y, make_float4((float)x, (float)y, (float)zlo, (float)zhi),
              make_float2((float)sx, (float)sy));
}
__device__ __forceinline__ uint32_t q8(double v, uint32_t& big) {
  const double r = rint(v);
  big |= (r > 120.0 || r < -120.0) ? 1u : 0u;
  return (uint32_t)((int)fmin(fmax(r, -120.0), 120.0) & 0xff);
}
__device__ __forceinline__ void put_rec_lig(const KParams& P, const Dev& d, uint2 h, int p, int w, int own, double cx,
                                            double cy, double cz, const double* sx, const double* sy,
                                            const double* sz) {
  uint32_t big = 0, b[9];
#pragma unroll
  for (int j = 0; j < 3; ++j) {
    b[3 * j] = q8(sx[j] - cx, big);
    b[3 * j + 1] = q8(sy[j] - cy, big);
    b[3 * j + 2] = q8(sz[j] - cz, big);
  }
  const uint32_t w0 = b[0] | b[1] << 8 | b[2] << 16 | b[3] << 24, w1 = b[4] | b[5] << 8 | b[6] << 16 | b[7] << 24,
                 w2 = b[8] | big << 8;
  put_rec_raw(P, d, h, p, w, 0, own, cx, cy, make_float4((float)cx, (float)cy, (float)cz, __uint_as_float(w0)),
              make_float2(__uint_as_float(w1), __uint_as_float(w2)));
}

__global__ void k_rec_check(KParams P, Dev d) {
  const uint32_t step = d.ctl->step;
  bool bad = false;
  for (int i = blockIdx.x * blockDim.x + threadIdx.x; i < 2 * P.N; i += gridDim.x * blockDim.x)
    bad |= d.rec_step[i] != step;
  if (__ballot(bad) && __lane_id() == 0) atomicOr(&d.ctl->err, ERR_RESOLVE);
}

__device__ __forceinline__ int rec_status(const KParams& P, const Dev& d, int p) {
// ... 1017 lines not shown
    else d.nxt.A2(m, row) = v;
  }
  if (nB > 1 && lane < csize) {
    const int e = L->res[lane];
    grow[lane] = L->slot[e < NA ? e : e - NA];
  }
}

__device__ __forceinline__ void cx_put_new(const KParams& P, const Dev& d, CxLds* L, int csize, int lane, int own,
                                           uint2 home, int st) {
  if (lane >= csize) return;
  const int m = L->slot[lane];
  const double* b = L->bead[lane];
  const int kind = m >= P.NA;
  bool ext = true;
  for (int j = 2; j <= 4; ++j) {
    const int o = (kind ? (j - 1) * 2 : (j - 1) * 4) * 3;
    const double ex = b[o] - b[0], ey = b[o + 1] - b[1];
    ext &= kind ? ex * ex + ey * ey <= 35.0 * 35.0 : ex * ex + ey * ey <= 0.09;
  }
  if (!ext) atomicOr(&d.ctl->err, ERR_GEOMETRY);
  double zl = b[2], zh = b[2], sx = 0.0, sy = 0.0;
  if (kind) {
    const double ux[3] = {b[2 * 3], b[4 * 3], b[6 * 3]}, uy[3] = {b[2 * 3 + 1], b[4 * 3 + 1], b[6 * 3 + 1]},
                 uz[3] = {b[2 * 3 + 2], b[4 * 3 + 2], b[6 * 3 + 2]};
    put_rec_lig(P, d, home, m, 1, own, b[0], b[1], b[2], ux, uy, uz);
    return;
  }
  {
    const double z1 = b[2], z2 = b[(4) * 3 + 2], z3 = b[(8) * 3 + 2], z4 = b[(12) * 3 + 2];
    zl = fmin(fmin(z1, z2), fmin(z3, z4));
    zh = fmax(fmax(z1, z2), fmax(z3, z4));
    sx = b[(2 * 4 + 2) * 3];
    sy = b[(2 * 4 + 2) * 3 + 1];
  }
  put_rec(P, d, home, m, 1, st, own, b[0], b[1], zl, zh, sx, sy);
}

struct Bead0 {
  double x, y, z;
  bool ok;
};
template <bool LDS>
__device__ __forceinline__ Bead0 cx_bead0(const KParams& P, const Dev& d, CxLds* L, const int* grow, int csize, int lane) {
  const int ql = lane >> 4, bj = ((lane >> 2) & 3) + 1, bk = (lane & 3) + 1;
  Bead0 b{0.0, 0.0, 0.0, false};
  if (ql < csize) {
    const int m = LDS ? L->slot[ql] : grow[ql];
    if (bk <= (m < P.NA ? 4 : 2)) {
      b.x = d.cur.P(m, bj, bk, 0);
      b.y = d.cur.P(m, bj, bk, 1);
      b.z = d.cur.P(m, bj, bk, 2);
      b.ok = true;
    }
  }
  return b;
}
template <bool LDS>
__device__ __forceinline__ void cx_rigid(const KParams& P, const Dev& d, CxLds* L, const int* grow, int csize, int nB,
                                         uint32_t rootid, uint32_t step, int lane, Bead0 b0) {
  const int NA = P.NA;
  const int nA = csize - nB;
  auto mslot = [&](int q) { return LDS ? L->slot[q] : grow[q]; };
  double u0, u1, u2, u3;
  kmcr::uniform2(P.key, kmcr::DOM_DIFF, rootid, 0, step, 0, &u0, &u1);
  kmcr::uniform2(P.key, kmcr::DOM_DIFF, rootid, 0, step, 1, &u2, &u3);
  double amp = (nB == 1 ? P.amp_bond : 0.0) * u0;
  double phai = u1 * 2 * P.pai;
  double dx = amp * kmcm::cos(phai), dy = amp * kmcm::sin(phai);
  const int ql = lane >> 4, bj = ((lane >> 2) & 3) + 1, bk = (lane & 3) + 1;
  const int npass = (csize + 3) >> 2;
  auto load = [&](int q, double& x, double& y, double& z) -> bool {
    if (q >= csize) return false;
    const int m = mslot(q);
    if (bk > (m < NA ? 4 : 2)) return false;
    x = d.cur.P(m, bj, bk, 0);
    y = d.cur.P(m, bj, bk, 1);
    z = d.cur.P(m, bj, bk, 2);
    return true;
  };
  const double c0x = b0.x, c0y = b0.y, c0z = b0.z;
  const bool c0 = b0.ok;
  auto bead = [&](int ps, double& x, double& y, double& z) -> bool {
    if (ps == 0) {
      x = c0x;
      y = c0y;
      z = c0z;
      return c0;
    }
    return load(ps * 4 + ql, x, y, z);
  };
  double PBx = 0, PBy = 0;
  for (int ps = 0; ps < npass; ++ps) {
    double x = 0, y = 0, z = 0;
    bead(ps, x, y, z);
    const double vx = x + dx, vy = y + dy;
    const int cnt = min(4, csize - ps * 4);
    for (int s = 0; s < cnt; ++s) {
      PBx = PBx + __shfl(vx, s * 16, 64);
      PBy = PBy + __shfl(vy, s * 16, 64);
    }
  }
  PBx = P.box_x * kmcm::round_(PBx / (nA + nB) / P.box_x);
  PBy = P.box_y * kmcm::round_(PBy / (nA + nB) / P.box_y);
  double cmx = 0, cmy = 0, cmz = 0;
  for (int ps = 0; ps < npass; ++ps) {
    double x = 0, y = 0, z = 0;
    bead(ps, x, y, z);
    const double ax = (x + dx) - PBx, ay = (y + dy) - PBy;
    const int cnt = min(4, csize - ps * 4);
    for (int s = 0; s < cnt; ++s)
#pragma unroll
      for (int j = 0; j < 4; ++j) {
        cmx = cmx + __shfl(ax, s * 16 + j * 4, 64);
        cmy = cmy + __shfl(ay, s * 16 + j * 4, 64);
        cmz = cmz + __shfl(z, s * 16 + j * 4, 64);
      }
  }
  cmx = cmx / (4 * nA + 4 * nB);
  cmy = cmy / (4 * nA + 4 * nB);
  cmz = cmz / (4 * nA + 4 * nB);
  Rot t = euler(0, 0, (2 * u2 - 1) * (nB == 1 ? P.rot_bond : 0.0));
  for (int ps = 0; ps < npass; ++ps) {
    double x = 0, y = 0, z = 0;
    if (!bead(ps, x, y, z)) continue;
    const int q = ps * 4 + ql, m = mslot(q);
    double ox = (x + dx) - PBx;
    double oy = (y + dy) - PBy;
    double oz = z;
    const double nx = rx(t, ox, oy, oz, cmx, cmy, cmz), ny = ry(t, ox, oy, oz, cmx, cmy, cmz),
                 nz = rz(t, ox, oy, oz, cmx, cmy, cmz);
    if (LDS) {
      double* b = &L->bead[q][((bj - 1) * (m < NA ? 4 : 2) + (bk - 1)) * 3];
      b[0] = nx;
      b[1] = ny;
      b[2] = nz;
    } else {
      d.nxt.P(m, bj, bk, 0) = nx;
      d.nxt.P(m, bj, bk, 1) = ny;
      d.nxt.P(m, bj, bk, 2) = nz;
    }
  }
}

#define CXP 16

__device__ __forceinline__ bool cx_current(const Dev& d, int4 desc) {
  return d.cx_alive[desc.x] == 1u && d.cx_off[desc.x] == desc.y;
}

#ifndef CXP_BATCH
#define CXP_BATCH 4
#endif
__device__ __forceinline__ void cx_params(const KParams& P, const Dev& d, uint32_t first, uint32_t stride) {
  const uint32_t n = d.ctl->n_cx, step = d.ctl->step;
  for (uint32_t c = first; c < n; c += stride) {
    const int4 desc = d.cx_list[c];
    if (!cx_current(d, desc)) continue;
    const int csize = desc.z & 0xffff, nB = desc.z >> 16, nA = csize - nB;
    if (csize > CXL) {
      d.cx_heavy[atomicAdd(&d.ctl->n_heavy, 1u)] = desc;
      continue;
    }
    double u0, u1, u2, u3;
    const uint32_t rk = rkey(P, d, desc.w);
    kmcr::uniform2(P.key, kmcr::DOM_DIFF, rk, 0, step, 0, &u0, &u1);
    kmcr::uniform2(P.key, kmcr::DOM_DIFF, rk, 0, step, 1, &u2, &u3);
    double amp = (nB == 1 ? P.amp_bond : 0.0) * u0;
    double phai = u1 * 2 * P.pai;
    double dx = amp * kmcm::cos(phai), dy = amp * kmcm::sin(phai);
    const int* row = d.members + desc.y;
    double PBx = 0, PBy = 0, cmx = 0, cmy = 0, cmz = 0;
    for (int pass = 0; pass < 2; ++pass) {
      for (int t0 = 0; t0 < csize; t0 += CXP_BATCH) {
        double2 xy[CXP_BATCH][4];
        double z[CXP_BATCH][4];
#pragma unroll
        for (int i = 0; i < CXP_BATCH; ++i) {
          const int t = t0 + i;
          if (t >= csize) break;
          const int m = row[t];
          if (pass == 0) {
            xy[i][0] = m < P.NA ? d.cur.Axy(m, 1, 1) : d.cur.Bxy(m - P.NA, 1, 1);
          } else {
#pragma unroll
            for (int j = 0; j < 4; ++j) {
              xy[i][j] = m < P.NA ? d.cur.Axy(m, j + 1, 1) : d.cur.Bxy(m - P.NA, j + 1, 1);
              z[i][j] = d.cur.P(m, j + 1, 1, 2);
            }
          }
        }
#pragma unroll
        for (int i = 0; i < CXP_BATCH; ++i) {
          if (t0 + i >= csize) break;
          if (pass == 0) {
            PBx = PBx + (xy[i][0].x + dx);
            PBy = PBy + (xy[i][0].y + dy);
          } else {
#pragma unroll
            for (int j = 0; j < 4; ++j) {
              cmx = cmx + ((xy[i][j].x + dx) - PBx);
              cmy = cmy + ((xy[i][j].y + dy) - PBy);
              cmz = cmz + z[i][j];
            }
          }
        }
      }
      if (pass == 0) {
        PBx = P.box_x * kmcm::round_(PBx / (nA + nB) / P.box_x);
        PBy = P.box_y * kmcm::round_(PBy / (nA + nB) / P.box_y);
      }
    }
    cmx = cmx / (4 * nA + 4 * nB);
    cmy = cmy / (4 * nA + 4 * nB);
    cmz = cmz / (4 * nA + 4 * nB);
    const Rot t = euler(0, 0, (2 * u2 - 1) * (nB == 1 ? P.rot_bond : 0.0));
    double* o = d.cxp + (size_t)desc.x * CXP;
    o[0] = dx;
    o[1] = dy;
    o[2] = PBx;
    o[3] = PBy;
    o[4] = cmx;
    o[5] = cmy;
    o[6] = cmz;
#pragma unroll
    for (int a = 0; a < 3; ++a)
#pragma unroll
      for (int b = 0; b < 3; ++b) o[7 + a * 3 + b] = t.t[a][b];
  }
}

template <bool IS_A>
__device__ __forceinline__ void move_member(const KParams& P, const Dev& d, int i, const double* cp, int root) {
  constexpr int NK = IS_A ? 4 : 2, ROWS = IS_A ? ROWS_A : ROWS_B;
  const int n = IS_A ? P.NA : P.NB, p = IS_A ? i : P.NA + i;
  const double2* src = reinterpret_cast<const double2*>(IS_A ? d.cur.a : d.cur.b);
  double2* dst = reinterpret_cast<double2*>(IS_A ? d.nxt.a : d.nxt.b);
  double2 r[ROWS];
#pragma unroll
  for (int w = 0; w < ROWS; ++w) r[w] = ld_r(src[bead_elem(i, w, n, ROWS)]);
  const double dx = cp[0], dy = cp[1], PBx = cp[2], PBy = cp[3], cmx = cp[4], cmy = cp[5], cmz = cp[6];
  Rot t;
#pragma unroll
  for (int a = 0; a < 3; ++a)
#pragma unroll
    for (int b = 0; b < 3; ++b) t.t[a][b] = cp[7 + a * 3 + b];
  const uint2 h = d.home[p];
  const int st = rec_status(P, d, p), own = d.owner[p];
  auto recs = [&](int w) {
    if constexpr (IS_A)
      put_rec(P, d, h, p, w, st, own, r[0].x, r[0].y, fmin(fmin(r[16].x, r[16].y), fmin(r[20].x, r[20].y)),
              fmax(fmax(r[16].x, r[16].y), fmax(r[20].x, r[20].y)), r[10].x, r[10].y);
    else {
      const double ux[3] = {r[2].x, r[4].x, r[6].x}, uy[3] = {r[2].y, r[4].y, r[6].y},
                   uz[3] = {r[8].y, r[10].x, r[10].y};
      put_rec_lig(P, d, h, p, w, own, r[0].x, r[0].y, r[8].x, ux, uy, uz);
    }
  };
  recs(0);
#pragma unroll
  for (int jp = 0; jp < 2; ++jp)
#pragma unroll
    for (int k = 0; k < NK; ++k) {
      const int r1 = 2 * jp * NK + k, r2 = (2 * jp + 1) * NK + k, rzr = 4 * NK + jp * NK + k;
      const double z1 = r[rzr].x, z2 = r[rzr].y;
      const double ox1 = (r[r1].x + dx) - PBx, oy1 = (r[r1].y + dy) - PBy;
      const double ox2 = (r[r2].x + dx) - PBx, oy2 = (r[r2].y + dy) - PBy;
      r[r1] = make_double2(rx(t, ox1, oy1, z1, cmx, cmy, cmz), ry(t, ox1, oy1, z1, cmx, cmy, cmz));
      r[r2] = make_double2(rx(t, ox2, oy2, z2, cmx, cmy, cmz), ry(t, ox2, oy2, z2, cmx, cmy, cmz));
      r[rzr] = make_double2(rz(t, ox1, oy1, z1, cmx, cmy, cmz), rz(t, ox2, oy2, z2, cmx, cmy, cmz));
    }
#pragma unroll
  for (int w = 0; w < ROWS; ++w) st_n(dst[bead_elem(i, w, n, ROWS)], r[w]);
  recs(1);
  bool ext = true;
#pragma unroll
  for (int j = 1; j < 4; ++j) {
    const double ex = r[j * NK].x - r[0].x, ey = r[j * NK].y - r[0].y;
    ext &= IS_A ? ex * ex + ey * ey <= 0.09 : ex * ex + ey * ey <= 35.0 * 35.0;
  }
  if (!ext) atomicOr(&d.cx_ext[root - P.NA], 1u);
}

#ifndef CXCHECK_BATCH
#define CXCHECK_BATCH 1
#endif
__global__ void __launch_bounds__(256) k_cx_check(KParams P, Dev d) {
  const int NA = P.NA, NB = P.NB;
  const uint32_t n = d.ctl->n_cx;
  const Beads& N = d.nxt;
  for (uint32_t c = blockIdx.x * blockDim.x + threadIdx.x; c < n; c += gridDim.x * blockDim.x) {
    const int4 desc = d.cx_list[c];
    if (!cx_current(d, desc)) continue;
    const int csize = desc.z & 0xffff, nB = desc.z >> 16;
    if (csize > CXL) continue;
    const uint32_t xb = d.cx_ext[desc.x & CXD_LB];
    if (xb) d.cx_ext[desc.x & CXD_LB] = 0u;
    bool heavy = nB != 1;
#if CXCHECK_BATCH
    if (!heavy) {
      const int lb = desc.x;
      int a1r[3], a2r[3];
#pragma unroll
      for (int j = 0; j < 3; ++j) a1r[j] = B_NEI(d, lb, j + 2);
      heavy = N.B(lb, 1, 2, 2) != (N.B(lb, 1, 1, 2) + P.rb);
#pragma unroll
      for (int j = 0; j < 3; ++j) a2r[j] = A_NEI3(d, a1r[j] > 0 ? a1r[j] - 1 : 0);
      bool mis[3];
#pragma unroll
      for (int j = 0; j < 3; ++j) mis[j] = bond_misaligned(P, N, lb, j + 2, a1r[j] > 0 ? a1r[j] - 1 : 0);
#pragma unroll
      for (int j = 0; j < 3; ++j) {
        const bool cm = cis_misaligned(P, N, a1r[j] > 0 ? a1r[j] - 1 : 0, a2r[j] > 0 ? a2r[j] - 1 : 0);
        heavy |= a1r[j] > 0 && (mis[j] || (a2r[j] != 0 && cm));
      }
    }
#else
    if (!heavy) {
      const int lb = desc.x;
      heavy = N.B(lb, 1, 2, 2) != (N.B(lb, 1, 1, 2) + P.rb);
#pragma unroll
      for (int j = 2; j <= 4; ++j) {
        const int a1ref = B_NEI(d, lb, j);
        if (a1ref == 0) continue;
        const int a1 = a1ref - 1, a2ref = A_NEI3(d, a1);
        heavy |= bond_misaligned(P, N, lb, j, a1) || (a2ref != 0 && cis_misaligned(P, N, a1, a2ref - 1));
      }
    }
#endif
    if (heavy) {
      d.cx_heavy[atomicAdd(&d.ctl->n_heavy, 1u)] = make_int4(desc.x | CXD_MOVED, desc.y, desc.z, desc.w);
      continue;
    }
    if (xb) atomicOr(&d.ctl->err, ERR_GEOMETRY);
  }
}

#ifndef HEAVY_WAVES
#define HEAVY_WAVES 2
#endif
__global__ void __launch_bounds__(256, HEAVY_WAVES) k_complex_heavy(KParams P, Dev d) {
  __shared__ CxLds lds[4];
  const int lane = __lane_id(), NA = P.NA, NB = P.NB;
  CxLds* L = &lds[threadIdx.x >> 6];
  const uint32_t step = d.ctl->step;
  auto global_path = [&](int lb) {
    const int csize = d.cx_size[lb], nB = d.cx_nb[lb];
    const int* brow = d.members + d.cx_off[lb];
    int* grow = d.shuf + d.cx_off[lb];
    for (int q = lane; q < csize; q += 64) grow[q] = brow[q];
    if (lane == 0) d.shuf_tag[lb] = step;
    wave_sync();
    cx_rigid<false>(P, d, L, grow, csize, nB, rkey(P, d, d.id_of[NA + lb]), step, lane,
                    cx_bead0<false>(P, d, L, grow, csize, lane));
    wave_sync();
    if (lane == 0) {
      int pA = -1;
      for (int q = csize - 1; q >= 0 && pA < 0; --q)
        if (grow[q] < NA) pA = grow[q];
      CxT<Beads, GlbLinks> X{P, step, rkey(P, d, d.id_of[NA + lb]), grow, csize, d.nxt, GlbLinks{&d, NA, NB, step},
                             &d.ctl->err};
      complex_align(X, nB, lb, pA);
    }
    wave_sync();
    for (int q = lane; q < csize; q += 64) put_recs_glb(P, d, grow[q]);
  };
  if (blockIdx.x == 0 && threadIdx.x < 64) {
    const uint32_t no = d.ctl->n_overflow;
    for (uint32_t o = 0; o < no; ++o) {
      int lb = lane == 0 ? bfs_overflow_one(P, d, o) : -1;
      lb = __shfl(lb, 0, 64);
      wave_sync();
      if (lb >= 0) global_path(lb);
    }
  }
  const uint32_t n = d.ctl->n_heavy;
  const uint32_t w = (blockIdx.x * blockDim.x + threadIdx.x) >> 6, nw = (gridDim.x * blockDim.x) >> 6;
  for (uint32_t c = w; c < n; c += nw) {
#ifdef KMC_STAMPS
    uint64_t t0_ = Stamper::now(), t_ = t0_;
#define CXS(i)                                                                                   \
  do {                                                                                           \
    if (lane == 0) {                                                                             \
      const uint64_t v_ = Stamper::now();                                                        \
      atomicAdd((unsigned long long*)&d.ctl->stamps[16 + (i)], (unsigned long long)(v_ - t_)); \
      t_ = v_;                                                                                   \
    }                                                                                            \
  } while (0)
#else
#define CXS(i)
#endif
    const int4 desc = d.cx_heavy[c];
    const int lb = desc.x & CXD_LB;
    if (!(desc.x & CXD_MOVED)) {
      global_path(lb);
      continue;
    }
    const int csize = desc.z & 0xffff, nB = desc.z >> 16;
    const int mslot = cx_stage_mrec(d, L, desc.y, csize, NA, lane);
    uint2 mhome = make_uint2(0u, 0u);
    int mst = 0;
    if (mslot >= 0) {
      mhome = d.home[mslot];
      mst = rec_status(P, d, mslot);
    }
    wave_sync();
    cx_load_beads(d, L, csize, NA, lane);
    if (nB > 1)
      for (int e = lane; e < CX_SHUF * CXL; e += 64) {
        const int call = e / CXL, pos = e % CXL;
        if (pos >= 1 && pos < csize - 1)
          L->rnd[call][pos] = kmcr::rand31(P.key, kmcr::DOM_SHUF, rkey(P, d, desc.w), call, step, pos);
      }
    wave_sync();
    CXS(0);
    {
      const uint64_t rm = __ballot(lane < csize && L->slot[lane] < NA);
      const int pA = rm ? 63 - __clzll((long long)rm) : -1;
      CxT<LdsBeads, LdsLinks> X{P, step, rkey(P, d, desc.w), L->res, csize, LdsBeads{L}, LdsLinks{L, NA}, &d.ctl->err,
                                L->rnd};
      if (P.cx_serial) {
        if (lane == 0) complex_align(X, nB, 0, pA);
        wave_sync();
      } else {
        complex_align_wave(X, L, nB, pA, lane);
      }
    }
    CXS(1);
    cx_write_back(d, L, d.shuf + desc.y, csize, nB, NA, lane);
    if (nB > 1 && lane == 0) d.shuf_tag[lb] = step;
    CXS(2);
    cx_put_new(P, d, L, csize, lane, desc.w, mhome, mst);
    wave_sync();
    CXS(3);
#ifdef KMC_STAMPS
    if (lane == 0) {
      atomicAdd((unsigned long long*)&d.ctl->stamps[20], 1ull);
      atomicMax((unsigned long long*)&d.ctl->stamps[21], (unsigned long long)(t_ - t0_));
      atomicAdd((unsigned long long*)&d.ctl->stamps[22], (unsigned long long)csize);
    }
#endif
#undef CXS
  }
}

__device__ __forceinline__ void propose_one(const KParams& P, const Dev& d, int p) {
  if (p >= P.N) return;
  const uint32_t step = d.ctl->step;
  const int NA = P.NA;
  uint8_t k = d.ukind[p];
  if (k == U_FREE_A) {
    propose_free_a(P, d, p, step);
  } else if (k == U_DIMER) {
    const int q = A_NEI3(d, p) - 1;
    propose_dimer(P, d, p, q, step);
  } else if (k == U_FREE_B) {
    propose_free_b(P, d, p - P.NA, p, step);
  }
}

#ifndef MEMBER_WAVES
#define MEMBER_WAVES 1
#endif
__global__ void __launch_bounds__(256, MEMBER_WAVES) k_move_members(KParams P, Dev d) {
  const int p = blockIdx.x * blockDim.x + threadIdx.x, NA = P.NA;
  if (p >= P.N) return;
  const int r = d.croot[p];
  if (r < 0 || (r & CROOT_BIG)) return;
  const double* cp = d.cxp + (size_t)(r - NA) * CXP;
  if (p < NA) move_member<true>(P, d, p, cp, r);
  else move_member<false>(P, d, p - NA, cp, r);
}

#ifndef FREE_WAVES
#define FREE_WAVES 1
#endif
__global__ void __launch_bounds__(256, FREE_WAVES) k_propose_free(KParams P, Dev d, int gC) {
  if ((int)blockIdx.x < gC) {
    cx_params(P, d, blockIdx.x * blockDim.x + threadIdx.x, (uint32_t)gC * blockDim.x);
    return;
  }
  propose_one(P, d, (int)((blockIdx.x - gC) * blockDim.x + threadIdx.x));
}

struct Own {
  double x[4], y[4], z[4];
  bool isA;
};
__device__ __forceinline__ void load_own(const KParams& P, const Beads& B, int m, Own& o) {
  o.isA = m < P.NA;
  double2 z12, z34;
  if (o.isA) {
#pragma unroll
    for (int k = 0; k < 4; ++k) {
      const double2 xy = B.Axy(m, k + 1, 1);
      o.x[k] = xy.x;
      o.y[k] = xy.y;
    }
    z12 = B.A2(m, 16);
    z34 = B.A2(m, 20);
  } else {
    int b = m - P.NA;
#pragma unroll
    for (int k = 0; k < 4; ++k) {
      const double2 xy = B.Bxy(b, k + 1, 1);
      o.x[k] = xy.x;
      o.y[k] = xy.y;
    }
    z12 = B.B2(b, 8);
    z34 = B.B2(b, 10);
  }
  o.z[0] = z12.x;
  o.z[1] = z12.y;
  o.z[2] = z34.x;
  o.z[3] = z34.y;
}

__device__ bool exact_collide(const KParams& P, const Own& o, const Beads& B, int q) {
  const int NA = P.NA;
  const bool qA = q < NA;
  if (o.isA && qA) {
    const double2 xy = B.Axy(q, 1, 1), z12 = B.A2(q, 16);
    const double dx = xy.x - o.x[0], dy = xy.y - o.y[0], dz = z12.x - o.z[0];
    return d2(dx, dy, dz) < P.T_aa;
  }
  double qx[4], qy[4], qz[4];
  double2 z12, z34;
  if (qA) {
#pragma unroll
    for (int j = 0; j < 4; ++j) {
      const double2 xy = B.Axy(q, j + 1, 1);
      qx[j] = xy.x;
      qy[j] = xy.y;
    }
    z12 = B.A2(q, 16);
    z34 = B.A2(q, 20);
  } else {
    const int b = q - NA;
    qx[0] = qy[0] = 0.0;
#pragma unroll
    for (int j = 1; j < 4; ++j) {
      const double2 xy = B.Bxy(b, j + 1, 1);
      qx[j] = xy.x;
      qy[j] = xy.y;
    }
    z12 = B.B2(b, 8);
    z34 = B.B2(b, 10);
  }
  qz[0] = z12.x;
  qz[1] = z12.y;
  qz[2] = z34.x;
  qz[3] = z34.y;
  bool hit = false;
  if (o.isA) {
#pragma unroll
    for (int j = 1; j < 4; ++j)
#pragma unroll
      for (int k = 0; k < 4; ++k) hit |= d2(qx[j] - o.x[k], qy[j] - o.y[k], qz[j] - o.z[k]) < P.T_ab;
  } else if (!qA) {
#pragma unroll
    for (int j = 1; j < 4; ++j)
#pragma unroll
      for (int k = 1; k < 4; ++k) hit |= d2(qx[j] - o.x[k], qy[j] - o.y[k], qz[j] - o.z[k]) < P.T_bb;
  } else {
#pragma unroll
    for (int j = 0; j < 4; ++j)
#pragma unroll
      for (int k = 1; k < 4; ++k) hit |= d2(qx[j] - o.x[k], qy[j] - o.y[k], qz[j] - o.z[k]) < P.T_ab;
  }
  return hit;
}

__device__ __forceinline__ bool prefilter(bool mA, float mx, float my, float mzl, float mzh, bool qA, float4 r) {
  float dx = r.x - mx, dy = r.y - my;
  float dxy2 = dx * dx + dy * dy;
  float dz = r.z - mzl;
  bool same = dxy2 + dz * dz < (mA ? 42.0f * 42.0f : 131.5f * 131.5f);
  float lz = mA ? r.z : mzl, alo = mA ? mzl : r.z, ahi = mA ? mzh : r.w;
  bool mixed = (dxy2 < 86.5f * 86.5f) & (lz > alo - 86.5f) & (lz < ahi + 86.5f);
  return mA == qA ? same : mixed;
}

#ifndef PAIR_PK
#define PAIR_PK 1
#endif
typedef float pk2 __attribute__((ext_vector_type(2)));
__device__ __forceinline__ bool prefilter_d(bool mA, float mzl, float mzh, bool qA, float4 r, float dxy2) {
  const float dz = r.z - mzl;
  const bool same = dxy2 + dz * dz < (mA ? 42.0f * 42.0f : 131.5f * 131.5f);
  const float lz = mA ? r.z : mzl, alo = mA ? mzl : r.z, ahi = mA ? mzh : r.w;
  const bool mixed = (dxy2 < 86.5f * 86.5f) & (lz > alo - 86.5f) & (lz < ahi + 86.5f);
  return mA == qA ? same : mixed;
}

#define EBUF 128
struct WgList {
  int2 buf[EBUF];
  uint32_t n;
  uint32_t base;
};

__device__ __forceinline__ void wg_list_init(WgList& L) {
  if (threadIdx.x == 0) L.n = 0;
  __syncthreads();
}

__device__ __forceinline__ int my_shard() { return blockIdx.x & (NSHARD - 1); }

__device__ __forceinline__ bool sl_push(const SList& s, int2 v, uint32_t* err) {
  const int k = my_shard();
  const uint32_t pos = wave_slot(&s.cnt[k]);
  if (pos < s.cap) {
    s.data[(size_t)k * s.cap + pos] = v;
    return true;
  }
  atomicOr(err, ERR_EDGES);
  return false;
}

__device__ __forceinline__ uint32_t sl_total(const SList& s) {
  uint32_t t = 0;
  for (int k = 0; k < NSHARD; ++k) t += min(s.cnt[k], s.cap);
  return t;
}

__device__ __forceinline__ int2 sl_get(const SList& s, uint32_t t) {
  int k = 0;
  for (; k < NSHARD - 1; ++k) {
    const uint32_t c = min(s.cnt[k], s.cap);
    if (t < c) break;
    t -= c;
  }
  return s.data[(size_t)k * s.cap + t];
}

// ... 1435 lines not shown
      int i = d.slot_of[(int)(key >> 34)], q = d.slot_of[(int)((key >> 2) & 0xffffffffu)];
      uint32_t fl = (uint32_t)(key & 3);
      bool unb = A_ST2(d, i) == 0 && A_ST2(d, q) == 0;
      bool ok = pass == 0 ? (unb && (fl & 1)) : (!unb && (fl & 2) && A_ST3(d, i) == 0 && A_ST3(d, q) == 0);
      if (ok) e[atomicAdd(&m, 1u)] = key & ~3ull;
    }
    __syncthreads();
    uint32_t n = m;
    auto apply = [&](uint64_t key) {
      int i = d.slot_of[(int)(key >> 34)], q = d.slot_of[(int)((key >> 2) & 0xffffffffu)];
      if (P.dd) dd_xbond(d, (int)(key >> 34), (int)((key >> 2) & 0xffffffffu));
      A_ST3(d, i) = 1;
      A_ST3(d, q) = 1;
      A_NEI3(d, q) = i + 1;
      A_NEI3(d, i) = q + 1;
      mark_bond_change(P, d, i, d.ctl->step);
      mark_bond_change(P, d, q, d.ctl->step);
    };
    if (n > 0 && n <= SMALL_EDGES) {
      uint64_t key = 0;
      if (small_greedy(n, e, CisV{}, acc, &key)) apply(key);
    } else if (n > 0) {
      uint32_t np = pow2ceil(n);
      for (uint32_t t = n + threadIdx.x; t < np; t += blockDim.x) e[t] = ~0ull;
      __syncthreads();
      block_sort(e, np);
      block_greedy(n, e, CisV{}, d.ent, d.gi32, acc, &d.ctl->err);
      for (uint32_t t = threadIdx.x; t < n; t += blockDim.x)
        if (acc[t]) apply(e[t]);
    }
    __syncthreads();
  }
}

__device__ __forceinline__ bool cis_diss(const KParams& P, const Dev& d, int i, int q, bool mono, uint32_t step) {
  const int NA = P.NA;
  uint32_t dom = mono ? kmcr::DOM_MD : kmcr::DOM_CD;
  double pd = mono ? P.p_mdiss : P.p_cdiss;
  double ui = kmcr::uniform(P.key, dom, rkey(P, d, d.id_of[i]), 0, step, 0);
  double uq = kmcr::uniform(P.key, dom, rkey(P, d, d.id_of[q]), 0, step, 0);
  if (ui < pd || uq < pd) {
    A_ST3(d, i) = 0;
    A_ST3(d, q) = 0;
    A_NEI3(d, i) = 0;
    A_NEI3(d, q) = 0;
    mark_bond_change(P, d, i, step);
    mark_bond_change(P, d, q, step);
    return true;
  }
  return false;
}

__global__ void __launch_bounds__(1024) k_match(KParams P, Dev d) {
  rl_match(P, d);
  __syncthreads();
  cis_match(P, d);
}

__device__ __forceinline__ bool rl_breaks(const KParams& P, const Dev& d, int i, uint32_t step) {
  return kmcr::uniform(P.key, kmcr::DOM_RLD, rkey(P, d, d.id_of[i]), 0, step, 0) < P.p_diss;
}

__device__ __forceinline__ int wave_sum(int v) {
  for (int off = 32; off > 0; off >>= 1) v += __shfl_down(v, off, 64);
  return v;
}
__device__ __forceinline__ int wave_max(int v) {
  for (int off = 32; off > 0; off >>= 1) {
    int o = __shfl_down(v, off, 64);
    v = o > v ? o : v;
  }
  return v;
}

template <int DISS_PER>
__global__ void __launch_bounds__(256) k_diss_observe(KParams P, Dev d) {
  const int NA = P.NA, NB = P.NB;
  __shared__ int red[4][6];
  const uint32_t step = d.ctl->step;
  int v[6] = {0, 0, 0, 0, 0, 0};
  const int p0 = blockIdx.x * blockDim.x * DISS_PER + threadIdx.x;
  int st2[DISS_PER], st3[DISS_PER];
  uint8_t kind[DISS_PER];
#pragma unroll
  for (int k = 0; k < DISS_PER; ++k) {
    const int p = p0 + k * (int)blockDim.x;
    st2[k] = 0;
    st3[k] = 0;
    kind[k] = U_NONE;
    if (p < NA) {
      st2[k] = A_ST2(d, p);
      st3[k] = A_ST3(d, p);
    } else if (p < P.N) {
      kind[k] = d.ukind[p];
    }
  }
#pragma unroll
  for (int k = 0; k < DISS_PER; ++k) {
    const int p = p0 + k * (int)blockDim.x;
    if (p < NA) {
      const int i = p;
      int st2_i = st2[k];
      if (st2_i == 1 && rl_breaks(P, d, i, step)) {
        int q = A_NEI2(d, i) - 1, kk = A_NEI4(d, i);
        int lb = q - NA;
        A_ST2(d, i) = 0;
        B_ST(d, lb, kk) = 0;
        A_NEI2(d, i) = 0;
        A_NEI4(d, i) = 0;
        B_NEI(d, lb, kk) = 0;
        mark_bond_change(P, d, i, step);
        mark_bond_change(P, d, q, step);
        st2_i = 0;
      }
      v[0] += dd_owned(P, d, d.id_of[i]) ? st2_i : 0;
      if (st3[k] == 1) {
        int q = A_NEI3(d, i) - 1;
        if (i < q) {
          int st2_q = A_ST2(d, q);
          if (st2_q == 1 && rl_breaks(P, d, q, step)) st2_q = 0;
          const bool mono = st2_i == 0 && st2_q == 0;
          if (!cis_diss(P, d, i, q, mono, step)) v[mono ? 1 : 2] += dd_owned(P, d, min(d.id_of[i], d.id_of[q])) ? 1 : 0;
        }
      }
    } else if (p < P.N) {
      uint8_t kd = kind[k];
      if (!dd_owned(P, d, d.id_of[p])) kd = U_NONE;
      if (kd == U_COMPLEX) {
        int sz = d.cx_size[p - NA];
        v[3] += sz;
        v[4] += 1;
        v[5] = max(v[5], sz);
      } else if (kd == U_FREE_B) {
        v[5] = max(v[5], 1);
      }
    }
  }
  for (int f = 0; f < 5; ++f) v[f] = wave_sum(v[f]);
  v[5] = wave_max(v[5]);
  int w = threadIdx.x >> 6;
  if ((threadIdx.x & 63) == 0)
    for (int f = 0; f < 6; ++f) red[w][f] = v[f];
  __syncthreads();
  if (threadIdx.x < 6) {
    int f = threadIdx.x, a = red[0][f];
    for (int ww = 1; ww < 4; ++ww) a = f == 5 ? max(a, red[ww][f]) : a + red[ww][f];
    d.obs_part[blockIdx.x * 8 + f] = a;
  }
}

__global__ void __launch_bounds__(1024) k_finalize(KParams P, Dev d, double time_step, int nblk) {
  __shared__ int red[16][6];
  __shared__ uint32_t tot[5];
  if (threadIdx.x < 5) tot[threadIdx.x] = 0;
  int v[6] = {0, 0, 0, 0, 0, 0};
#pragma unroll 4
  for (int b = threadIdx.x; b < nblk; b += blockDim.x) {
    const int4 lo = *(const int4*)&d.obs_part[b * 8];
    const int2 hi = *(const int2*)&d.obs_part[b * 8 + 4];
    v[0] += lo.x;
    v[1] += lo.y;
    v[2] += lo.z;
    v[3] += lo.w;
    v[4] += hi.x;
    v[5] = max(v[5], hi.y);
  }
  for (int f = 0; f < 5; ++f) v[f] = wave_sum(v[f]);
  v[5] = wave_max(v[5]);
  if ((threadIdx.x & 63) == 0)
    for (int f = 0; f < 6; ++f) red[threadIdx.x >> 6][f] = v[f];
  __syncthreads();
  for (int k = threadIdx.x; k < 5 * NSHARD; k += blockDim.x) {
    const int l = k / NSHARD;
    const uint32_t cap = l == 0 ? d.cand.cap : l == 1 ? d.conf.cap : l == 2 ? d.plist.cap : l == 3 ? d.rej.cap : d.pairs.cap;
    atomicAdd(&tot[l], min(d.shard_cnt[k], cap));
    d.shard_cnt[k] = 0;
  }
  const uint32_t fstep = d.ctl->step;
  const uint32_t ff = (d.ctl->cx_cursor > P.cx_limit || d.ctl->n_dirty[fstep & 1] > (uint32_t)P.N) ? 1u : 0u;
  if (P.NB > 0) {
    if (ff) {
      cx_reset_all(P, d, threadIdx.x, blockDim.x);
    } else {
      cx_dissolve_dirty(P, d, fstep);
      if (threadIdx.x == 0) d.ctl->full_now = 0;
    }
  }
  __syncthreads();
  if (threadIdx.x != 0) return;
  for (int w = 1; w < (int)(blockDim.x >> 6); ++w)
    for (int f = 0; f < 6; ++f) red[0][f] = f == 5 ? max(red[0][f], red[w][f]) : red[0][f] + red[w][f];
  Ctl* c = d.ctl;
  const uint32_t step = c->step, obs_idx = c->obs_idx, n_rl = c->n_rl, n_cisc = c->n_cisc, n_ovf = c->n_overflow;
  const int32_t off_rl = c->off_rl, off_mono = c->off_mono, off_cis = c->off_cis, off_bond = c->off_bond;
  const int32_t rl = red[0][0], mono = red[0][1], cis = red[0][2], tot_prot = red[0][3], tot_clu = red[0][4];
  const int32_t maxc = max(c->maxc, red[0][5]);
  kmc_obs_dev o;
  o.step = (int64_t)step;
  o.t = (double)(int)step * time_step;
  o.rl = rl + off_rl;
  o.mono = mono + off_mono;
  o.cis = cis + off_cis;
  o.bond = (rl + mono + cis) + off_bond;
  o.cluster_size = tot_clu != 0 ? (double)tot_prot / tot_clu : 0.0;
  o.maxc = maxc;
  o.tot_prot = tot_prot;
  o.tot_clu = tot_clu;
  o.reserved = 0;
  d.obs[obs_idx] = o;
  if (c->err && c->err_step == 0) {
    c->err_step = step;
    c->err_first = c->err;
  }
  c->n_forced += ff;
  c->maxc = maxc;
  c->obs_idx = obs_idx + 1;
  c->step = step + 1;
  for (int k = 0; k < 5; ++k) c->last[k] = tot[k];
  c->last[5] = n_rl;
  c->last[6] = n_cisc;
  c->last[7] = n_ovf;
  c->last_outl = c->n_outl;
  c->n_overflow = 0;
  c->n_dirty[(step + 1) & 1] = 0;
  c->n_heavy = 0;
  c->n_pend = 0;
  c->n_pqu = 0;
  c->n_pqe = 0;
  c->n_rl = 0;
  c->n_cisc = 0;
  c->n_outl = 0;
  c->n_dense = 0;
}


__device__ __forceinline__ uint32_t slot_key(const KParams& P, double x, double y) {
  return (uint32_t)cell_y(P, y) * (uint32_t)P.ncx + (uint32_t)cell_x(P, x);
}

__global__ void k_slot_keys(KParams P, Dev d, uint64_t* keys, int32_t* vals, int group, int ob, int kb) {
  int s = blockIdx.x * blockDim.x + threadIdx.x;
  if (s >= P.N) return;
  int lead = s, own = d.id_of[s];
  if (group) {
    const int o = d.owner[s];
    if (o >= 0 && o < P.N) {
      lead = d.slot_of[o];
      own = o;
    }
  }
  double x = d.cur.P(lead, 1, 1, 0), y = d.cur.P(lead, 1, 1, 1);
  const int tb = group == 2 ? 1 : 0;
  const uint64_t cx = group == 2 && d.croot[s] >= 0 ? 1ull : 0ull;
  const uint64_t kind = s >= P.NA ? 1ull : 0ull;
  keys[s] = kind << (ob + kb + tb) | cx << (ob + kb) | (uint64_t)slot_key(P, x, y) << ob |
            (uint64_t)(group ? (uint32_t)own : 0u);
  vals[s] = s < P.NA ? s : s - P.NA;
}

#define RS_TILE 4096
#define SCAN_TILE 4096

__device__ __forceinline__ uint64_t rs_peers(uint32_t dg, uint64_t live) {
  uint64_t m = live;
#pragma unroll
  for (int b = 0; b < 8; ++b) {
    const uint64_t v = __ballot((dg >> b) & 1u);
    m &= (dg >> b) & 1u ? v : ~v;
  }
  return m;
}

__global__ void __launch_bounds__(256) k_rs_hist(const uint64_t* __restrict__ keys, int n, int shift,
                                                 int32_t* __restrict__ cnt, int nblk) {
  __shared__ int h[256];
  h[threadIdx.x] = 0;
  __syncthreads();
  const int lane = __lane_id();
  const uint64_t lt = (1ull << lane) - 1ull;
  const size_t base = (size_t)blockIdx.x * RS_TILE;
  for (int j = threadIdx.x; j < RS_TILE; j += 256) {
    const size_t i = base + j;
    const bool ok = i < (size_t)n;
    const uint32_t dg = ok ? (uint32_t)(keys[i] >> shift) & 255u : 0u;
    const uint64_t pe = rs_peers(dg, __ballot(ok));
    if (ok && (pe & lt) == 0) atomicAdd(&h[dg], __popcll(pe));
  }
  __syncthreads();
  cnt[(size_t)threadIdx.x * nblk + blockIdx.x] = h[threadIdx.x];
}

__device__ __forceinline__ int block_excl_256(int x, int* sh, int& total) {
  const int lane = __lane_id(), w = threadIdx.x >> 6;
  int inc = x;
#pragma unroll
  for (int o = 1; o < 64; o <<= 1) {
    const int t = __shfl_up(inc, o, 64);
    if (lane >= o) inc += t;
  }
  if (lane == 63) sh[w] = inc;
  __syncthreads();
  int off = 0;
  total = 0;
#pragma unroll
  for (int q = 0; q < 4; ++q) {
    const int c = sh[q];
    off += q < w ? c : 0;
    total += c;
  }
  __syncthreads();
  return off + inc - x;
}
__global__ void __launch_bounds__(256) k_rs_rows(int32_t* __restrict__ cnt, int nblk, int32_t* __restrict__ tot) {
  __shared__ int sh[4];
  int32_t* row = cnt + (size_t)blockIdx.x * nblk;
  int carry = 0;
  for (int b0 = 0; b0 < nblk; b0 += 256) {
    const int i = b0 + (int)threadIdx.x;
    const int x = i < nblk ? row[i] : 0;
    int t;
    const int e = block_excl_256(x, sh, t);
    if (i < nblk) row[i] = carry + e;
    carry += t;
  }
  if (threadIdx.x == 0) tot[blockIdx.x] = carry;
}

__global__ void __launch_bounds__(256) k_rs_scatter(const uint64_t* __restrict__ kin, const int32_t* __restrict__ vin,
                                                    uint64_t* __restrict__ kout, int32_t* __restrict__ vout, int n,
                                                    int shift, const int32_t* __restrict__ cnt,
                                                    const int32_t* __restrict__ tot, int nblk) {
  __shared__ int wc[4][256];
  __shared__ int gb[256], ts[256], sh[4];
  __shared__ uint64_t sk[RS_TILE];
  __shared__ int32_t sv[RS_TILE];
  const int lane = __lane_id(), w = threadIdx.x >> 6, t = threadIdx.x;
  for (int i = t; i < 4 * 256; i += 256) (&wc[0][0])[i] = 0;
  {
    int all;
    const int db = block_excl_256(tot[t], sh, all);
    gb[t] = db + cnt[(size_t)t * nblk + blockIdx.x];
  }
  __syncthreads();
  const size_t base = (size_t)blockIdx.x * RS_TILE + (size_t)w * (RS_TILE / 4);
  const uint64_t lt = (1ull << lane) - 1ull;
  constexpr int C = RS_TILE / 256;
  uint64_t k[C];
  int32_t v[C], r[C];
#pragma unroll
  for (int c = 0; c < C; ++c) {
    const size_t i = base + (size_t)c * 64 + lane;
    k[c] = i < (size_t)n ? kin[i] : 0ull;
    v[c] = i < (size_t)n ? vin[i] : 0;
  }
#pragma unroll
  for (int c = 0; c < C; ++c) {
    const bool ok = base + (size_t)c * 64 + lane < (size_t)n;
    const uint32_t dg = (uint32_t)(k[c] >> shift) & 255u;
    const uint64_t pe = rs_peers(dg, __ballot(ok));
    const int prior = ok ? wc[w][dg] : 0;
    r[c] = prior + __popcll(pe & lt);
    if (ok && (pe & ~lt & ~(1ull << lane)) == 0) wc[w][dg] = prior + __popcll(pe);
  }
  __syncthreads();
  {
    int run = 0;
#pragma unroll
// ... 135 lines not shown
```

Before: 2.220 billion.

## Chain steps by reclassifying only dirty particles and fusing BFS into propose

Adds a step-chain mode, on by default when the side stream is off and B particles exist. The per-step full classify pass is replaced by incremental reclassification of dirty particles inside k_finalize, which also logs kind changes. BFS complex registration and complex parameter computation are fused into the k_propose_free launch, and the separate cx_check kernel is dropped by checking moved geometry inline and routing failures to the heavy path. This removes several full-N kernel launches and passes per step. In exchange it adds more single-block serial work in finalize and more shared-memory and register pressure in the fused propose kernel.

Result: faster. 2.351 billion, median of 6 (+5.9%).

```diff
diff --git a/kmc-with-a-diffusion-reaction-algorithm_amd/csrc/kmc_device.h b/kmc-with-a-diffusion-reaction-algorithm_amd/csrc/kmc_device.h
--- a/kmc-with-a-diffusion-reaction-algorithm_amd/csrc/kmc_device.h
+++ b/kmc-with-a-diffusion-reaction-algorithm_amd/csrc/kmc_device.h
@@ -33,6 +33,9 @@
   int dbg_recs;
   int dbg_cand;
   int dd;
+  int step_chain;
+  int dbg_classify;
+  int dbg_counts;
 };
 
 struct Ctl {
@@ -63,6 +66,9 @@
   uint64_t vtag;
   uint64_t stamps[24];
   uint32_t dd_xcol, dd_xbond;
+  uint32_t n_ulog, n_reclass;
+  uint32_t n_cx0, n_bfs_reg, n_chk_heavy;
+  uint32_t n_cx1;
 };
 
 #define DD_JCAP 256
diff --git a/kmc-with-a-diffusion-reaction-algorithm_amd/csrc/kmc_engine.hip b/kmc-with-a-diffusion-reaction-algorithm_amd/csrc/kmc_engine.hip
--- a/kmc-with-a-diffusion-reaction-algorithm_amd/csrc/kmc_engine.hip
+++ b/kmc-with-a-diffusion-reaction-algorithm_amd/csrc/kmc_engine.hip
@@ -381,6 +381,8 @@
   rc |= dalloc(s, &d.cx_alive, NB);
   rc |= dalloc(s, &d.bfs_cand, NB);
   rc |= dalloc(s, &d.dlist, 2 * (size_t)N);
+  rc |= dalloc(s, &d.ulog, (size_t)N + NB);
+  rc |= dalloc(s, &d.cx_slot, NB);
   rc |= dalloc(s, &d.pend, N);
   rc |= dalloc(s, &d.ccnt, N);
   rc |= dalloc(s, &d.overflow, NB);
@@ -419,6 +421,7 @@
   s->poison = po && *po == '1';
   const char* dc = getenv("KMC_DEBUG_COUNTS");
   s->debug_counts = dc && *dc == '1';
+  K.dbg_counts = s->debug_counts;
   const char* dsy = getenv("KMC_DEBUG_SYNC");
   s->debug_sync = dsy && *dsy == '1';
   const char* pc = getenv("KMC_DEBUG_PAIR_CHUNK");
@@ -441,6 +444,10 @@
     s->use_graphs = gr && *gr == '1';
     const char* cs = getenv("KMC_CX_STREAM");
     s->cx_stream = (cs && *cs) ? std::max(0, std::min(3, atoi(cs))) : ((int64_t)N >= CX_STREAM_N ? 3 : 0);
+    const char* sc = getenv("KMC_STEP_CHAIN");
+    K.step_chain = !(sc && *sc == '0') && s->cx_stream == 0 && NB > 0 && (int64_t)N < (1ll << ULOG_SHIFT);
+    const char* dcl = getenv("KMC_DEBUG_CLASSIFY");
+    K.dbg_classify = dcl && *dcl == '1';
     const char* cpw = getenv("KMC_CX_PARAMS_WG");
     s->cx_params_wg = cpw && *cpw ? std::max(0, atoi(cpw)) : 0;
     const char* ht = getenv("KMC_DEBUG_HTAG");
@@ -935,17 +942,23 @@
     (void)hipMemsetAsync(d.nxt.a, 0xff, sizeof(double) * 48 * bead_slots(K.NA), st);
     (void)hipMemsetAsync(d.nxt.b, 0xff, sizeof(double) * 24 * bead_slots(K.NB), st);
   }
-  if (K.NB > 0 && (s->need_full || re_sort || s->always_full))
-    TIMED(KI_CX_KILL, (k_cx_kill<<<std::min(gN, 1024), T, 0, st>>>(K, d)));
+  const bool full = s->need_full || re_sort || s->always_full;
+  if (K.NB > 0 && full) TIMED(KI_CX_KILL, (k_cx_kill<<<std::min(gN, 1024), T, 0, st>>>(K, d)));
   s->need_full = false;
   const int per = K.N >= COARSE_N ? 4 : 1, gP = (K.N + T * per - 1) / (T * per);
-  if (per == 4) TIMED(KI_CLASSIFY, (k_classify<4><<<gP, T, 0, st>>>(K, d)));
-  else TIMED(KI_CLASSIFY, (k_classify<1><<<gP, T, 0, st>>>(K, d)));
+  if (!(K.step_chain && !K.dd) || full) {
+    if (per == 4) TIMED(KI_CLASSIFY, (k_classify<4><<<gP, T, 0, st>>>(K, d)));
+    else TIMED(KI_CLASSIFY, (k_classify<1><<<gP, T, 0, st>>>(K, d)));
+  } else if (K.dbg_classify) {
+    if (per == 4) k_classify_check<4><<<gP, T, 0, st>>>(K, d);
+    else k_classify_check<1><<<gP, T, 0, st>>>(K, d);
+  }
   {
     Bracket b_(s, KI_PROPOSE, st);
     const int gL = std::min(2048, (K.NB + T - 1) / T);
     const bool side = s->cx_stream != 0 && K.NB > 0 && !s->use_graphs;
-    if (K.NB > 0 && (!side || s->cx_stream == 3)) {
+    const bool chain = K.step_chain && !K.dd;
+    if (K.NB > 0 && !chain && (!side || s->cx_stream == 3)) {
       TIMED(KI_BFS, (k_bfs<<<gB, T, 0, st>>>(K, d)));
     }
     const int gC = K.NB > 0 ? std::min(gL, 512) : 0;
@@ -954,14 +967,14 @@
       const int rc = side_stream(s);
       if (rc != KMC_OK) return rc;
       hipStream_t sd = s->side;
-      k_propose_free<<<gP3, T, 0, st>>>(K, d, gP3);
+      k_propose_free<0><<<gP3, T, 0, st>>>(K, d, gP3, 0);
       TIMED(KI_MOVE_MEMBERS, (k_move_members<<<gN, T, 0, st>>>(K, d)));
       HIPCHK(s, hipEventRecord(s->ev_fork, st));
       HIPCHK(s, hipStreamWaitEvent(sd, s->ev_fork, 0));
       TIMED_ON(KI_CX_CHECK, sd, (k_cx_check<<<gL, T, 0, sd>>>(K, d)));
       TIMED_ON(KI_CX_HEAVY, sd, (k_complex_heavy<<<1024, T, 0, sd>>>(K, d)));
       HIPCHK(s, hipEventRecord(s->ev_join, sd));
-      TIMED(KI_PROPOSE_FREE, (k_propose_free<<<gN, T, 0, st>>>(K, d, 0)));
+      TIMED(KI_PROPOSE_FREE, (k_propose_free<0><<<gN, T, 0, st>>>(K, d, 0, 0)));
       HIPCHK(s, hipStreamWaitEvent(st, s->ev_join, 0));
     } else if (side) {
       const int rc = side_stream(s);
@@ -970,14 +983,14 @@
       HIPCHK(s, hipEventRecord(s->ev_fork, st));
       HIPCHK(s, hipStreamWaitEvent(sd, s->ev_fork, 0));
       TIMED_ON(KI_BFS, sd, (k_bfs<<<gB, T, 0, sd>>>(K, d)));
-      k_propose_free<<<gC, T, 0, sd>>>(K, d, gC);
+      k_propose_free<0><<<gC, T, 0, sd>>>(K, d, gC, 0);
       if (s->cx_stream == 1) {
         TIMED_ON(KI_MOVE_MEMBERS, sd, (k_move_members<<<gN, T, 0, sd>>>(K, d)));
         TIMED_ON(KI_CX_CHECK, sd, (k_cx_check<<<gL, T, 0, sd>>>(K, d)));
         TIMED_ON(KI_CX_HEAVY, sd, (k_complex_heavy<<<1024, T, 0, sd>>>(K, d)));
       }
       HIPCHK(s, hipEventRecord(s->ev_join, sd));
-      TIMED(KI_PROPOSE_FREE, (k_propose_free<<<gN, T, 0, st>>>(K, d, 0)));
+      TIMED(KI_PROPOSE_FREE, (k_propose_free<0><<<gN, T, 0, st>>>(K, d, 0, 0)));
       HIPCHK(s, hipStreamWaitEvent(st, s->ev_join, 0));
       if (s->cx_stream == 2) {
         TIMED(KI_MOVE_MEMBERS, (k_move_members<<<gN, T, 0, st>>>(K, d)));
@@ -985,10 +998,12 @@
         TIMED(KI_CX_HEAVY, (k_complex_heavy<<<1024, T, 0, st>>>(K, d)));
       }
     } else {
-      TIMED(KI_PROPOSE_FREE, (k_propose_free<<<gC + gN, T, 0, st>>>(K, d, gC)));
+      const int gF = chain ? gB : 0;
+      if (chain) TIMED(KI_PROPOSE_FREE, (k_propose_free<1><<<gF + gC + gN, T, 0, st>>>(K, d, gC, gF)));
+      else TIMED(KI_PROPOSE_FREE, (k_propose_free<0><<<gC + gN, T, 0, st>>>(K, d, gC, 0)));
       if (K.NB > 0) {
         TIMED(KI_MOVE_MEMBERS, (k_move_members<<<gN, T, 0, st>>>(K, d)));
-        TIMED(KI_CX_CHECK, (k_cx_check<<<gL, T, 0, st>>>(K, d)));
+        if (!chain) TIMED(KI_CX_CHECK, (k_cx_check<<<gL, T, 0, st>>>(K, d)));
         TIMED(KI_CX_HEAVY, (k_complex_heavy<<<1024, T, 0, st>>>(K, d)));
       }
     }
@@ -1205,9 +1220,10 @@
     s->clusters_valid = true;
     if (s->debug_counts) {
       const uint32_t* l = s->ctl_host->last;
-      fprintf(stderr, "kmc step %lld: candidates %u conflicts %u pending-units %u rejected %u rxn-pairs %u rl-edges %u cis-edges %u bfs-overflow %u outliers %u (list growth 2^%d, replays %lld, snapshots %lld, forced rebuilds %u)\n",
+      fprintf(stderr, "kmc step %lld: candidates %u conflicts %u pending-units %u rejected %u rxn-pairs %u rl-edges %u cis-edges %u bfs-overflow %u outliers %u (list growth 2^%d, replays %lld, snapshots %lld, forced rebuilds %u, reclassified %u, bfs-registered %u, params-heavy %u)\n",
               (long long)s->step_done, l[0], l[1], l[2], l[3], l[4], l[5], l[6], l[7], s->ctl_host->last_outl, s->grow,
-              (long long)s->n_replays, (long long)s->n_snapshots, s->ctl_host->n_forced);
+              (long long)s->n_replays, (long long)s->n_snapshots, s->ctl_host->n_forced, s->ctl_host->n_reclass,
+              s->ctl_host->n_bfs_reg, s->ctl_host->n_chk_heavy);
       if (s->K.dbg_cand) {
         const uint32_t* c = s->ctl_host->cand_kind;
         const uint32_t* r = s->ctl_host->rxn_kind;
@@ -1287,6 +1303,15 @@
   std::vector<int32_t> off(NB), size(NB), mem(N), id_of(N), slot_of(N);
   HIPCHK(s, hipStreamSynchronize(s->stream));
   HIPCHK(s, hipMemcpy(kind.data(), s->d.ukind, N, hipMemcpyDeviceToHost));
+  if (s->K.step_chain && !s->K.dd) {
+    std::vector<int32_t> ulog(std::min<size_t>(s->ctl_host->n_ulog, (size_t)N + NB));
+    if (!ulog.empty())
+      HIPCHK(s, hipMemcpy(ulog.data(), s->d.ulog, sizeof(int32_t) * ulog.size(), hipMemcpyDeviceToHost));
+    for (int pass = 0; pass < 2; ++pass)
+      for (const int32_t e : ulog)
+        if (((uint8_t)(e >> ULOG_SHIFT) == U_COMPLEX) == (pass == 1))
+          kind[e & ((1 << ULOG_SHIFT) - 1)] = (uint8_t)(e >> ULOG_SHIFT);
+  }
   HIPCHK(s, hipMemcpy(off.data(), s->d.cx_off, sizeof(int32_t) * NB, hipMemcpyDeviceToHost));
   HIPCHK(s, hipMemcpy(size.data(), s->d.cx_size, sizeof(int32_t) * NB, hipMemcpyDeviceToHost));
   std::vector<int32_t> shuf(s->d.mcap);
diff --git a/kmc-with-a-diffusion-reaction-algorithm_amd/csrc/kmc_kernels.hip b/kmc-with-a-diffusion-reaction-algorithm_amd/csrc/kmc_kernels.hip
--- a/kmc-with-a-diffusion-reaction-algorithm_amd/csrc/kmc_kernels.hip
+++ b/kmc-with-a-diffusion-reaction-algorithm_amd/csrc/kmc_kernels.hip
@@ -35,10 +35,12 @@
   uint32_t* cx_alive;
   uint32_t* bfs_cand;
   int32_t* dlist;
+  int32_t* ulog;
   uint32_t* pend;
   unsigned long long* ccnt;
   int32_t* overflow;
   int4* cx_list;
+  int32_t* cx_slot;
   int4* cx_heavy;
   uint2* home;
   int32_t* hstart;
@@ -171,9 +173,48 @@
   return (uint32_t)__shfl((int)base, leader, 64) + pre;
 }
 
-template <int CLASSIFY_PER>
-__global__ void k_classify(KParams P, Dev d) {
+__device__ __forceinline__ void classify_rule(const KParams& P, const Dev& d, int p, int n2, int n3, int s2, int r,
+                                              uint8_t& kind, int& ownkey) {
+  const int NA = P.NA;
+  kind = U_NONE;
+  int own = -1;
+  if (p < NA) {
+    const int i = p;
+    if (s2 == 0) {
+      kind = U_FREE_A;
+      own = p;
+    } else if (n2 == 0 && n3 != 0 && A_NEI3(d, n3 - 1) == i + 1 && A_NEI2(d, n3 - 1) == 0) {
+      int q = n3 - 1;
+      const bool lead = d.id_of[i] < d.id_of[q];
+      own = lead ? i : q;
+      kind = lead ? U_DIMER : U_DIMER_P;
+    }
+  } else if (n2 == 0 && n3 == 0 && s2 == 0) {
+    kind = U_FREE_B;
+    own = p;
+  }
+  if (r >= 0) {
+    own = r;
+    if (r == p) kind = U_COMPLEX;
+  }
+  ownkey = own < 0 ? -1 : d.id_of[own];
+}
+__device__ __forceinline__ void classify_links(const KParams& P, const Dev& d, int p, int& n2, int& n3, int& s2) {
   const int NA = P.NA, NB = P.NB;
+  if (p < NA) {
+    n2 = A_NEI2(d, p);
+    n3 = A_NEI3(d, p);
+    s2 = A_ST2(d, p) | A_ST3(d, p);
+  } else {
+    const int b = p - NA;
+    n2 = B_NEI(d, b, 2);
+    n3 = B_NEI(d, b, 3);
+    s2 = B_NEI(d, b, 4);
+  }
+}
+
+template <int CLASSIFY_PER, bool CHECK>
+__device__ __forceinline__ void classify_slots(const KParams& P, const Dev& d) {
   const int p0 = blockIdx.x * blockDim.x * CLASSIFY_PER + threadIdx.x;
   int n2[CLASSIFY_PER], n3[CLASSIFY_PER], s2[CLASSIFY_PER], r[CLASSIFY_PER];
 #pragma unroll
@@ -182,16 +223,7 @@
     n2[k] = n3[k] = s2[k] = 0;
     r[k] = -1;
     if (p >= P.N) continue;
-    if (p < NA) {
-      n2[k] = A_NEI2(d, p);
-      n3[k] = A_NEI3(d, p);
-      s2[k] = A_ST2(d, p) | A_ST3(d, p);
-    } else {
-      const int b = p - NA;
-      n2[k] = B_NEI(d, b, 2);
-      n3[k] = B_NEI(d, b, 3);
-      s2[k] = B_NEI(d, b, 4);
-    }
+    classify_links(P, d, p, n2[k], n3[k], s2[k]);
     r[k] = d.croot[p];
     if (r[k] >= 0) r[k] &= ~CROOT_BIG;
   }
@@ -199,30 +231,24 @@
   for (int k = 0; k < CLASSIFY_PER; ++k) {
     const int p = p0 + k * (int)blockDim.x;
     if (p >= P.N) continue;
-    uint8_t kind = U_NONE;
-    int own = -1;
-    if (p < NA) {
-      const int i = p;
-      if (s2[k] == 0) {
-        kind = U_FREE_A;
-        own = p;
-      } else if (n2[k] == 0 && n3[k] != 0 && A_NEI3(d, n3[k] - 1) == i + 1 && A_NEI2(d, n3[k] - 1) == 0) {
-        int q = n3[k] - 1;
-        const bool lead = d.id_of[i] < d.id_of[q];
-        own = lead ? i : q;
-        kind = lead ? U_DIMER : U_DIMER_P;
-      }
-    } else if (n2[k] == 0 && n3[k] == 0 && s2[k] == 0) {
-      kind = U_FREE_B;
-      own = p;
-    }
-    if (r[k] >= 0) {
-      own = r[k];
-      if (r[k] == p) kind = U_COMPLEX;
-    }
-    d.ukind[p] = kind;
-    d.owner[p] = own < 0 ? -1 : d.id_of[own];
-  }
+    uint8_t kind;
+    int ownkey;
+    classify_rule(P, d, p, n2[k], n3[k], s2[k], r[k], kind, ownkey);
+    if (CHECK) {
+      if (d.ukind[p] != kind || d.owner[p] != ownkey) atomicOr(&d.ctl->err, ERR_RESOLVE);
+    } else {
+      d.ukind[p] = kind;
+      d.owner[p] = ownkey;
+    }
+  }
+}
+template <int CLASSIFY_PER>
+__global__ void k_classify(KParams P, Dev d) {
+  classify_slots<CLASSIFY_PER, false>(P, d);
+}
+template <int CLASSIFY_PER>
+__global__ void k_classify_check(KParams P, Dev d) {
+  classify_slots<CLASSIFY_PER, true>(P, d);
 }
 
 __device__ __forceinline__ void cx_reset_all(const KParams& P, const Dev& d, uint32_t tid, uint32_t nt) {
@@ -231,11 +257,16 @@
   if (tid == 0) {
     d.ctl->cx_cursor = 0;
     d.ctl->n_cx = 0;
+    d.ctl->n_cx0 = 0;
     d.ctl->full_now = 1;
   }
 }
 __global__ void k_cx_kill(KParams P, Dev d) {
   cx_reset_all(P, d, blockIdx.x * blockDim.x + threadIdx.x, gridDim.x * blockDim.x);
+}
+__device__ __forceinline__ void cx_desc_kill(const Dev& d, int b) {
+  const uint32_t sl = (uint32_t)d.cx_slot[b];
+  if (sl < d.mcap / 2) d.cx_list[sl].y = -1;
 }
 __device__ __forceinline__ void cx_dissolve_dirty(const KParams& P, const Dev& d, uint32_t step) {
   const int NA = P.NA;
@@ -246,11 +277,77 @@
     const int r = d.croot[p] & ~CROOT_BIG;
     if (r < 0 || atomicExch(&d.cx_alive[r - NA], 0u) != 1u) continue;
     const int b = r - NA, off = d.cx_off[b], sz = d.cx_size[b];
+    cx_desc_kill(d, b);
     for (int i = 0; i < sz; ++i) {
       const int m = d.members[off + i];
       d.croot[m] = -1;
       if (m >= NA) d.bfs_cand[m - NA] = next;
     }
+  }
+}
+
+#define ULOG_SHIFT 28
+__device__ __forceinline__ void reclass_store(const Dev& d, int p, uint8_t kind, int ownkey, uint32_t* nlog) {
+  const uint8_t old = d.ukind[p];
+  const bool unit = old == U_FREE_B || old == U_COMPLEX || kind == U_FREE_B || kind == U_COMPLEX;
+  if (old != kind && unit) d.ulog[atomicAdd(nlog, 1u)] = p | (int)old << ULOG_SHIFT;
+  d.ukind[p] = kind;
+  d.owner[p] = ownkey;
+}
+__device__ __forceinline__ void reclass_one(const KParams& P, const Dev& d, int p, uint8_t& kind, int& ownkey) {
+  int n2, n3, s2;
+  classify_links(P, d, p, n2, n3, s2);
+  classify_rule(P, d, p, n2, n3, s2, -1, kind, ownkey);
+}
+__device__ __forceinline__ void cx_dissolve_reclass(const KParams& P, const Dev& d, uint32_t step, uint32_t* nlog,
+                                                    uint32_t* nrec) {
+  const int NA = P.NA, NB = P.NB;
+  const uint32_t li = step & 1, n = min(d.ctl->n_dirty[li], (uint32_t)P.N), next = step + 1;
+  const uint32_t half = blockDim.x / 2;
+  const bool upper = threadIdx.x >= half;
+  int p0 = -1, q0 = -1, o0 = -1, oq = -1;
+  uint8_t k0 = U_NONE, kq = U_NONE;
+  if (!upper) {
+    for (uint32_t t = threadIdx.x; t < n; t += half) {
+      const int p = d.dlist[(size_t)li * P.N + t];
+      if (p >= NA) d.bfs_cand[p - NA] = next;
+      const int r = d.croot[p] & ~CROOT_BIG;
+      if (r < 0 || atomicExch(&d.cx_alive[r - NA], 0u) != 1u) continue;
+      const int b = r - NA, off = d.cx_off[b], sz = d.cx_size[b];
+      cx_desc_kill(d, b);
+      d.ulog[atomicAdd(nlog, 1u)] = r | (int)U_COMPLEX << ULOG_SHIFT;
+      for (int i = 0; i < sz; ++i) {
+        const int m = d.members[off + i];
+        d.croot[m] = -1;
+        d.ukind[m] = U_NONE;
+        d.owner[m] = -1;
+        if (m >= NA) d.bfs_cand[m - NA] = next;
+      }
+      atomicAdd(nrec, (uint32_t)sz);
+    }
+  } else if (threadIdx.x - half < n) {
+    p0 = d.dlist[(size_t)li * P.N + (threadIdx.x - half)];
+    const int q = p0 < NA ? A_NEI3(d, p0) : 0;
+    reclass_one(P, d, p0, k0, o0);
+    if (q > 0) {
+      q0 = q - 1;
+      reclass_one(P, d, q0, kq, oq);
+    }
+  }
+  __syncthreads();
+  if (p0 >= 0) reclass_store(d, p0, k0, o0, nlog);
+  if (q0 >= 0) reclass_store(d, q0, kq, oq, nlog);
+  if (p0 >= 0) atomicAdd(nrec, q0 >= 0 ? 2u : 1u);
+  for (uint32_t t = half + threadIdx.x; t < n; t += blockDim.x) {
+    const int p = d.dlist[(size_t)li * P.N + t];
+    const int q = p < NA ? A_NEI3(d, p) : 0;
+    reclass_one(P, d, p, k0, o0);
+    reclass_store(d, p, k0, o0, nlog);
+    if (q > 0) {
+      reclass_one(P, d, q - 1, kq, oq);
+      reclass_store(d, q - 1, kq, oq, nlog);
+    }
+    atomicAdd(nrec, q > 0 ? 2u : 1u);
   }
 }
 
@@ -286,7 +383,7 @@
 #define CXD_LB 0x3fffffff
 
 template <int STRIDE = 1>
-__device__ __forceinline__ void register_complex(const KParams& P, const Dev& d, int p, const int* q, int qn) {
+__device__ __forceinline__ int4 register_complex(const KParams& P, const Dev& d, int p, const int* q, int qn) {
   const int NA = P.NA, NB = P.NB;
   uint32_t off = wave_alloc(&d.ctl->cx_cursor, (uint32_t)qn);
   if (off + qn > d.mcap) {
@@ -346,17 +443,17 @@
   d.ukind[p] = U_COMPLEX;
   const int4 desc = make_int4(b, (int)off, qn | nb << 16, rootid);
   const uint32_t slot = wave_slot(&d.ctl->n_cx);
+  d.cx_slot[b] = (int)slot;
   if (slot < d.mcap / 2) d.cx_list[slot] = desc;
   else atomicOr(&d.ctl->err, ERR_MEMBERS);
-}
-
-__global__ void __launch_bounds__(256) k_bfs(KParams P, Dev d) {
-  __shared__ int qs[BFS_QCAP * 256];
+  return desc;
+}
+
+__device__ __forceinline__ bool bfs_one(const KParams& P, const Dev& d, int b, int* qs, int4& desc) {
   const int NA = P.NA, NB = P.NB;
-  int b = blockIdx.x * blockDim.x + threadIdx.x;
-  if (b >= NB) return;
-  if (!d.ctl->full_now && d.bfs_cand[b] != d.ctl->step) return;
-  if (B_NEI(d, b, 2) == 0 && B_NEI(d, b, 3) == 0 && B_NEI(d, b, 4) == 0) return;
+  if (b >= NB) return false;
+  if (!d.ctl->full_now && d.bfs_cand[b] != d.ctl->step) return false;
+  if (B_NEI(d, b, 2) == 0 && B_NEI(d, b, 3) == 0 && B_NEI(d, b, 4) == 0) return false;
   int* q = qs + threadIdx.x;
   int p = NA + b;
   const int pid = d.id_of[p];
@@ -398,18 +495,24 @@
         }
         bloom |= bit;
         if (qn == BFS_QCAP) {
-          if (lower(qn) || (v >= NA && d.id_of[v] < pid)) return;
+          if (lower(qn) || (v >= NA && d.id_of[v] < pid)) return false;
           uint32_t s = atomicAdd(&d.ctl->n_overflow, 1u);
           d.overflow[s] = b;
-          return;
+          return false;
         }
         q[(qn++) * 256] = v;
       }
     }
     head += nb;
   }
-  if (lower(qn)) return;
-  register_complex<256>(P, d, p, q, qn);
+  if (lower(qn)) return false;
+  desc = register_complex<256>(P, d, p, q, qn);
+  return true;
+}
+__global__ void __launch_bounds__(256) k_bfs(KParams P, Dev d) {
+  __shared__ int qs[BFS_QCAP * 256];
+  int4 desc;
+  bfs_one(P, d, blockIdx.x * blockDim.x + threadIdx.x, qs, desc);
 }
 
 __device__ __forceinline__ int bfs_overflow_one(const KParams& P, const Dev& d, uint32_t o) {
@@ -1733,15 +1836,81 @@
 #ifndef CXP_BATCH
 #define CXP_BATCH 4
 #endif
-__device__ __forceinline__ void cx_params(const KParams& P, const Dev& d, uint32_t first, uint32_t stride) {
-  const uint32_t n = d.ctl->n_cx, step = d.ctl->step;
-  for (uint32_t c = first; c < n; c += stride) {
-    const int4 desc = d.cx_list[c];
-    if (!cx_current(d, desc)) continue;
+struct CxMove {
+  double dx, dy, PBx, PBy, cmx, cmy, cmz;
+  Rot t;
+};
+__device__ __forceinline__ void cx_move_bead(const CxMove& M, double x, double y, double z, double& nx, double& ny,
+                                             double& nz) {
+  const double ox = (x + M.dx) - M.PBx, oy = (y + M.dy) - M.PBy;
+  nx = rx(M.t, ox, oy, z, M.cmx, M.cmy, M.cmz);
+  ny = ry(M.t, ox, oy, z, M.cmx, M.cmy, M.cmz);
+  nz = rz(M.t, ox, oy, z, M.cmx, M.cmy, M.cmz);
+}
+__device__ __forceinline__ double dxy_(double ax, double ay, double bx, double by) {
+  const double dx = ax - bx, dy = ay - by;
+  return kmcm::sqrt_(dx * dx + dy * dy);
+}
+
+#define CX_EXT_HEAVY 2u
+
+__device__ __forceinline__ bool cx_check_moved(const KParams& P, const Dev& d, const CxMove& M, int lb) {
+  const int NA = P.NA, NB = P.NB;
+  const Beads& R = d.cur;
+  const int a1r0 = B_NEI(d, lb, 2), a1r1 = B_NEI(d, lb, 3), a1r2 = B_NEI(d, lb, 4);
+  {
+    const double2 xy1 = R.B2(lb, 0), xy2 = R.B2(lb, 1);
+    const double z1 = R.B(lb, 1, 1, 2), z2 = R.B(lb, 1, 2, 2);
+    double nx, ny, nz1, nz2;
+    cx_move_bead(M, xy1.x, xy1.y, z1, nx, ny, nz1);
+    cx_move_bead(M, xy2.x, xy2.y, z2, nx, ny, nz2);
+    if (nz2 != (nz1 + P.rb)) return true;
+  }
+#pragma unroll 1
+  for (int j = 0; j < 3; ++j) {
+    const int a1ref = j == 0 ? a1r0 : j == 1 ? a1r1 : a1r2;
+    if (a1ref <= 0) continue;
+    const int a1 = a1ref - 1, a2ref = A_NEI3(d, a1);
+    const double2 l1 = R.B2(lb, (j + 1) * 2), l2 = R.B2(lb, (j + 1) * 2 + 1);
+    const double lz1 = R.B(lb, j + 2, 1, 2), lz2 = R.B(lb, j + 2, 2, 2);
+    double2 axy[2];
+    double az[2];
+#pragma unroll
+    for (int k = 0; k < 2; ++k) {
+      axy[k] = R.A2(a1, 8 + k);
+      az[k] = R.A(a1, 3, k + 1, 2);
+    }
+    double lx1, ly1, lx2, ly2, ax[3], ay[3], nz;
+    cx_move_bead(M, l1.x, l1.y, lz1, lx1, ly1, nz);
+    cx_move_bead(M, l2.x, l2.y, lz2, lx2, ly2, nz);
+#pragma unroll
+    for (int k = 0; k < 2; ++k) cx_move_bead(M, axy[k].x, axy[k].y, az[k], ax[k], ay[k], nz);
+    const double dd2 = dxy_(lx2, ly2, ax[1], ay[1]);
+    const double dd1 = dxy_(lx1, ly1, ax[0], ay[0]);
+    if (bond_mis_d(P, dd1, dd2)) return true;
+    if (a2ref == 0) continue;
+    const int a2 = a2ref - 1;
+    const double2 c1 = R.A2(a2, 8), c3 = R.A2(a2, 10), a3 = R.A2(a1, 10);
+    const double cz1 = R.A(a2, 3, 1, 2), cz3 = R.A(a2, 3, 3, 2), az3 = R.A(a1, 3, 3, 2);
+    double x1, y1, x3, y3;
+    cx_move_bead(M, a3.x, a3.y, az3, ax[2], ay[2], nz);
+    cx_move_bead(M, c1.x, c1.y, cz1, x1, y1, nz);
+    cx_move_bead(M, c3.x, c3.y, cz3, x3, y3, nz);
+    const double cd2 = dxy_(ax[2], ay[2], x3, y3);
+    const double cd1 = dxy_(ax[0], ay[0], x1, y1);
+    if (!AreSame(cd1, P.cis_cut / 2 + P.ra + P.ra) || !AreSame(cd2, P.cis_cut / 2)) return true;
+  }
+  return false;
+}
+
+template <bool CHAIN>
+__device__ __forceinline__ void cx_params_one(const KParams& P, const Dev& d, const int4 desc, uint32_t step) {
+  {
     const int csize = desc.z & 0xffff, nB = desc.z >> 16, nA = csize - nB;
+    if (csize == 0) return;
     if (csize > CXL) {
       d.cx_heavy[atomicAdd(&d.ctl->n_heavy, 1u)] = desc;
-      continue;
+      return;
     }
     double u0, u1, u2, u3;
     const uint32_t rk = rkey(P, d, desc.w);
@@ -1808,6 +1977,24 @@
     for (int a = 0; a < 3; ++a)
 #pragma unroll
       for (int b = 0; b < 3; ++b) o[7 + a * 3 + b] = t.t[a][b];
+    if (CHAIN) {
+      bool heavy = nB != 1;
+      if (!heavy) heavy = cx_check_moved(P, d, CxMove{dx, dy, PBx, PBy, cmx, cmy, cmz, t}, desc.x);
+      if (heavy) {
+        d.cx_ext[desc.x] = CX_EXT_HEAVY;
+        d.cx_heavy[atomicAdd(&d.ctl->n_heavy, 1u)] = make_int4(desc.x | CXD_MOVED, desc.y, desc.z, desc.w);
+        if (P.dbg_counts) atomicAdd(&d.ctl->n_chk_heavy, 1u);
+      }
+    }
+  }
+}
+template <bool CHAIN>
+__device__ __forceinline__ void cx_params(const KParams& P, const Dev& d, uint32_t first, uint32_t stride) {
+  const uint32_t n = CHAIN ? d.ctl->n_cx0 : d.ctl->n_cx, step = d.ctl->step;
+  for (uint32_t c = first; c < n; c += stride) {
+    const int4 desc = d.cx_list[c];
+    if (CHAIN ? desc.y < 0 : !cx_current(d, desc)) continue;
+    cx_params_one<CHAIN>(P, d, desc, step);
   }
 }
 
@@ -1820,12 +2007,11 @@
   double2 r[ROWS];
 #pragma unroll
   for (int w = 0; w < ROWS; ++w) r[w] = ld_r(src[bead_elem(i, w, n, ROWS)]);
-  const double dx = cp[0], dy = cp[1], PBx = cp[2], PBy = cp[3], cmx = cp[4], cmy = cp[5], cmz = cp[6];
-  Rot t;
+  CxMove M{cp[0], cp[1], cp[2], cp[3], cp[4], cp[5], cp[6], Rot{}};
 #pragma unroll
   for (int a = 0; a < 3; ++a)
 #pragma unroll
-    for (int b = 0; b < 3; ++b) t.t[a][b] = cp[7 + a * 3 + b];
+    for (int b = 0; b < 3; ++b) M.t.t[a][b] = cp[7 + a * 3 + b];
   const uint2 h = d.home[p];
   const int st = rec_status(P, d, p), own = d.owner[p];
   auto recs = [&](int w) {
@@ -1844,12 +2030,12 @@
 #pragma unroll
     for (int k = 0; k < NK; ++k) {
       const int r1 = 2 * jp * NK + k, r2 = (2 * jp + 1) * NK + k, rzr = 4 * NK + jp * NK + k;
-      const double z1 = r[rzr].x, z2 = r[rzr].y;
-      const double ox1 = (r[r1].x + dx) - PBx, oy1 = (r[r1].y + dy) - PBy;
-      const double ox2 = (r[r2].x + dx) - PBx, oy2 = (r[r2].y + dy) - PBy;
-      r[r1] = make_double2(rx(t, ox1, oy1, z1, cmx, cmy, cmz), ry(t, ox1, oy1, z1, cmx, cmy, cmz));
-      r[r2] = make_double2(rx(t, ox2, oy2, z2, cmx, cmy, cmz), ry(t, ox2, oy2, z2, cmx, cmy, cmz));
-      r[rzr] = make_double2(rz(t, ox1, oy1, z1, cmx, cmy, cmz), rz(t, ox2, oy2, z2, cmx, cmy, cmz));
+      double x1, y1, z1, x2, y2, z2;
+      cx_move_bead(M, r[r1].x, r[r1].y, r[rzr].x, x1, y1, z1);
+      cx_move_bead(M, r[r2].x, r[r2].y, r[rzr].y, x2, y2, z2);
+      r[r1] = make_double2(x1, y1);
+      r[r2] = make_double2(x2, y2);
+      r[rzr] = make_double2(z1, z2);
     }
 #pragma unroll
   for (int w = 0; w < ROWS; ++w) st_n(dst[bead_elem(i, w, n, ROWS)], r[w]);
@@ -1957,6 +2143,17 @@
   }
   const uint32_t n = d.ctl->n_heavy;
   const uint32_t w = (blockIdx.x * blockDim.x + threadIdx.x) >> 6, nw = (gridDim.x * blockDim.x) >> 6;
+  if (P.step_chain && !P.dd) {
+    const uint32_t ncx = d.ctl->n_cx1, first = n < nw ? n : 0u;
+    if (w >= first)
+      for (uint32_t c = (w - first) * 64 + lane; c < ncx; c += (nw - first) * 64) {
+        const int4 desc = d.cx_list[c];
+        if ((desc.z & 0xffff) > CXL || !cx_current(d, desc)) continue;
+        const uint32_t xb = d.cx_ext[desc.x];
+        if (xb) d.cx_ext[desc.x] = 0u;
+        if (xb == 1u) atomicOr(&d.ctl->err, ERR_GEOMETRY);
+      }
+  }
   for (uint32_t c = w; c < n; c += nw) {
 #ifdef KMC_STAMPS
     uint64_t t0_ = Stamper::now(), t_ = t0_;
@@ -2046,6 +2243,7 @@
 __global__ void __launch_bounds__(256, MEMBER_WAVES) k_move_members(KParams P, Dev d) {
   const int p = blockIdx.x * blockDim.x + threadIdx.x, NA = P.NA;
   if (p >= P.N) return;
+  if (p == 0 && P.step_chain) d.ctl->n_cx1 = min(d.ctl->n_cx, d.mcap / 2);
   const int r = d.croot[p];
   if (r < 0 || (r & CROOT_BIG)) return;
   const double* cp = d.cxp + (size_t)(r - NA) * CXP;
@@ -2056,12 +2254,25 @@
 #ifndef FREE_WAVES
 #define FREE_WAVES 1
 #endif
-__global__ void __launch_bounds__(256, FREE_WAVES) k_propose_free(KParams P, Dev d, int gC) {
-  if ((int)blockIdx.x < gC) {
-    cx_params(P, d, blockIdx.x * blockDim.x + threadIdx.x, (uint32_t)gC * blockDim.x);
+template <int CHAIN>
+__global__ void __launch_bounds__(256, CHAIN ? 3 : FREE_WAVES) k_propose_free(KParams P, Dev d, int gC, int gB) {
+  if constexpr (CHAIN != 0) {
+    __shared__ int qs[BFS_QCAP * 256];
+    if ((int)blockIdx.x < gB) {
+      int4 desc;
+      if (bfs_one(P, d, blockIdx.x * blockDim.x + threadIdx.x, qs, desc)) {
+        if (P.dbg_counts) atomicAdd(&d.ctl->n_bfs_reg, 1u);
+        cx_params_one<true>(P, d, desc, d.ctl->step);
+      }
+      return;
+    }
+  }
+  const int bid = (int)blockIdx.x - (CHAIN ? gB : 0);
+  if (bid < gC) {
+    cx_params<CHAIN != 0>(P, d, bid * blockDim.x + threadIdx.x, (uint32_t)gC * blockDim.x);
     return;
   }
-  propose_one(P, d, (int)((blockIdx.x - gC) * blockDim.x + threadIdx.x));
+  propose_one(P, d, (int)((bid - gC) * blockDim.x + threadIdx.x));
 }
 
 struct Own {
@@ -3803,7 +4014,9 @@
 __global__ void __launch_bounds__(1024) k_finalize(KParams P, Dev d, double time_step, int nblk) {
   __shared__ int red[16][6];
   __shared__ uint32_t tot[5];
+  __shared__ uint32_t nlog, nrec;
   if (threadIdx.x < 5) tot[threadIdx.x] = 0;
+  if (threadIdx.x == 5) nlog = nrec = 0;
   int v[6] = {0, 0, 0, 0, 0, 0};
 #pragma unroll 4
   for (int b = threadIdx.x; b < nblk; b += blockDim.x) {
@@ -3829,15 +4042,27 @@
   }
   const uint32_t fstep = d.ctl->step;
   const uint32_t ff = (d.ctl->cx_cursor > P.cx_limit || d.ctl->n_dirty[fstep & 1] > (uint32_t)P.N) ? 1u : 0u;
+  const bool chain = P.step_chain && !P.dd && P.NB > 0;
   if (P.NB > 0) {
     if (ff) {
       cx_reset_all(P, d, threadIdx.x, blockDim.x);
     } else {
-      cx_dissolve_dirty(P, d, fstep);
+      if (chain) cx_dissolve_reclass(P, d, fstep, &nlog, &nrec);
+      else cx_dissolve_dirty(P, d, fstep);
       if (threadIdx.x == 0) d.ctl->full_now = 0;
     }
   }
   __syncthreads();
+  if (chain && ff) {
+    for (int p = threadIdx.x; p < P.N; p += blockDim.x) {
+      uint8_t kind;
+      int ownkey;
+      reclass_one(P, d, p, kind, ownkey);
+      reclass_store(d, p, kind, ownkey, &nlog);
+    }
+    if (threadIdx.x == 0) nrec = (uint32_t)P.N;
+    __syncthreads();
+  }
   if (threadIdx.x != 0) return;
   for (int w = 1; w < (int)(blockDim.x >> 6); ++w)
     for (int f = 0; f < 6; ++f) red[0][f] = f == 5 ? max(red[0][f], red[w][f]) : red[0][f] + red[w][f];
@@ -3864,6 +4089,9 @@
     c->err_first = c->err;
   }
   c->n_forced += ff;
+  c->n_ulog = nlog;
+  c->n_reclass += nrec;
+  c->n_cx0 = min(c->n_cx, d.mcap / 2);
   c->maxc = maxc;
   c->obs_idx = obs_idx + 1;
   c->step = step + 1;
```
